# alibaba/animate-anything

Hardware: AMD Instinct MI355X
Metric: UNet3D denoising steps/sec @16fx512x512 bs=1 (higher is better)
Workload: dtype fp16; 1 GPU; animate_anything_512_v1.02 UNet3D (1413M params, seeded random init), 16 frames x 512x512, pipeline bs=1 per GPU (CFG batch 2, 17 frames inside), DPM-Solver++ step, hipGraph=on; clips_per_gpu=1, clips=1, parallelism=clip-sharded x1, collective=none

## Files before the change

### animate_anything_amd/_lib.py

```python
from __future__ import annotations

import ctypes as C
import os

import torch

AA_F16, AA_BF16, AA_F32 = 0, 1, 2
AA_ACT_NONE, AA_ACT_SILU, AA_ACT_GELU, AA_ACT_QUICK_GELU = 0, 1, 2, 3


class AaConvGemm(C.Structure):
    _fields_ = [
        ("a0", C.c_void_p), ("a1", C.c_void_p), ("w", C.c_void_p), ("bias", C.c_void_p),
        ("rowvec", C.c_void_p), ("residual", C.c_void_p), ("out", C.c_void_p),
        ("c0", C.c_int32), ("c1", C.c_int32),
        ("n_img", C.c_int32), ("h_in", C.c_int32), ("w_in", C.c_int32), ("h_virt", C.c_int32),
        ("w_virt", C.c_int32), ("h_out", C.c_int32), ("w_out", C.c_int32),
        ("kh", C.c_int32), ("kw", C.c_int32), ("stride", C.c_int32), ("pad_h", C.c_int32), ("pad_w", C.c_int32),
        ("n_out", C.c_int32), ("n_pad", C.c_int32), ("k_pad", C.c_int32),
        ("rowvec_div", C.c_int32), ("ldo", C.c_int32), ("ldr", C.c_int32),
        ("act", C.c_int32), ("geglu", C.c_int32), ("bias_per_row", C.c_int32),
        ("dtype", C.c_int32), ("out_dtype", C.c_int32), ("out_scale", C.c_float), ("workspace", C.c_void_p), ("workspace_bytes", C.c_int64), ("k_order", C.c_int32), ("debug", C.c_int32), ("tile", C.c_int32), ("k_splits", C.c_int32), ("rowvec_ld", C.c_int32), ("acc_scale", C.c_float),
        ("out_sy", C.c_int32), ("out_sx", C.c_int32), ("out_oy", C.c_int32), ("out_ox", C.c_int32),
        ("ln_stats", C.c_void_p), ("ln_cols", C.c_void_p), ("ln_parts", C.c_int32), ("ln_eps", C.c_float),
        ("row_stats", C.c_void_p), ("row_stats_parts", C.c_int32), ("tickets_len", C.c_int32), ("tickets", C.c_void_p),
        ("row_coef", C.c_void_p), ("row_coef_eps", C.c_float), ("_reserved107", C.c_int32),
    ]


class AaGroupNorm(C.Structure):
    _fields_ = [
        ("x0", C.c_void_p), ("x1", C.c_void_p), ("gamma", C.c_void_p), ("beta", C.c_void_p), ("y", C.c_void_p),
        ("c0", C.c_int32), ("c1", C.c_int32), ("n_groups_img", C.c_int32), ("tokens_per_group", C.c_int32),
        ("num_groups", C.c_int32), ("silu", C.c_int32), ("dtype", C.c_int32), ("eps", C.c_float),
    ]


class AaAttnOperand(C.Structure):
    _fields_ = [
        ("ptr", C.c_void_p), ("outer_stride", C.c_int64), ("inner_stride", C.c_int64), ("pos_stride", C.c_int64),
        ("ld", C.c_int32), ("col0", C.c_int32), ("outer_div", C.c_int32), ("seq_mod", C.c_int32),
    ]


class AaAttention(C.Structure):
    _fields_ = [
        ("q", AaAttnOperand), ("k", AaAttnOperand), ("v", AaAttnOperand), ("o", AaAttnOperand),
        ("n_outer", C.c_int32), ("n_inner", C.c_int32), ("heads", C.c_int32), ("head_dim", C.c_int32),
        ("q_len", C.c_int32), ("kv_len", C.c_int32), ("dtype", C.c_int32), ("scale", C.c_float), ("causal", C.c_int32), ("_pad", C.c_int32),
    ]


class AaSeqSelfAttn(C.Structure):
    _fields_ = [
        ("x", C.c_void_p), ("w", C.c_void_p), ("w_bias", C.c_void_p), ("pre_w", C.c_void_p), ("pre_bias", C.c_void_p), ("pre_residual", C.c_void_p), ("pre_out", C.c_void_p), ("o", C.c_void_p),
        ("outer_stride", C.c_int64), ("inner_stride", C.c_int64), ("pos_stride", C.c_int64), ("x_bytes", C.c_int64), ("o_bytes", C.c_int64),
        ("n_outer", C.c_int32), ("n_inner", C.c_int32), ("seq_len", C.c_int32), ("channels", C.c_int32), ("ldx", C.c_int32), ("ldo", C.c_int32), ("ld_res", C.c_int32), ("ld_pre", C.c_int32),
        ("normalize", C.c_int32), ("ln_eps", C.c_float), ("scale", C.c_float), ("dtype", C.c_int32), ("flags", C.c_int32),
    ]


class AaFFFused(C.Structure):
    _fields_ = [
        ("x", C.c_void_p), ("outer", C.c_void_p), ("out", C.c_void_p), ("w", C.c_void_p), ("rows", C.c_int64),
        ("channels", C.c_int32), ("ldx", C.c_int32), ("ld_outer", C.c_int32), ("ldo", C.c_int32),
        ("normalize", C.c_int32), ("ln_eps", C.c_float), ("dtype", C.c_int32), ("flags", C.c_int32),
    ]


class AaLinearRows(C.Structure):
    _fields_ = [
        ("x", C.c_void_p), ("residual", C.c_void_p), ("out", C.c_void_p), ("w", C.c_void_p), ("rows", C.c_int64),
        ("channels", C.c_int32), ("n_out", C.c_int32), ("ldx", C.c_int32), ("ld_res", C.c_int32), ("ldo", C.c_int32),
        ("normalize", C.c_int32), ("ln_eps", C.c_float), ("dtype", C.c_int32), ("flags", C.c_int32),
        ("row_affine", C.c_void_p), ("rows_per_group", C.c_int32), ("_pad", C.c_int32),
    ]


class AaQuantRowsFp8(C.Structure):
    _fields_ = [
        ("x", C.c_void_p), ("gamma", C.c_void_p), ("beta", C.c_void_p), ("q", C.c_void_p), ("scale", C.c_void_p), ("rows", C.c_int64),
        ("channels", C.c_int32), ("ldx", C.c_int32), ("ldq", C.c_int32), ("ln_eps", C.c_float), ("dtype", C.c_int32), ("_pad", C.c_int32),
    ]


class AaLinearFp8(C.Structure):
    _fields_ = [
        ("a", C.c_void_p), ("a_scale", C.c_void_p), ("w", C.c_void_p), ("w_scale", C.c_void_p), ("bias", C.c_void_p),
        ("residual", C.c_void_p), ("out", C.c_void_p), ("rows", C.c_int64),
        ("n", C.c_int32), ("k", C.c_int32), ("ld_res", C.c_int32), ("ldo", C.c_int32), ("geglu", C.c_int32), ("dtype", C.c_int32),
    ]


class AaDpmStep(C.Structure):
    _fields_ = [
        ("eps_uncond", C.c_void_p), ("eps_text", C.c_void_p), ("latents", C.c_void_p), ("x0_prev", C.c_void_p),
        ("latents_lp", C.c_void_p), ("n", C.c_int64),
        ("guidance", C.c_float), ("sigma_s", C.c_float), ("alpha_s", C.c_float),
        ("c_x", C.c_float), ("c_d0", C.c_float), ("c_d1", C.c_float), ("dtype", C.c_int32),
    ]


class AaPackLatents(C.Structure):
    _fields_ = [
        ("sample", C.c_void_p), ("cond", C.c_void_p), ("mask", C.c_void_p), ("out", C.c_void_p),
        ("batch", C.c_int32), ("sample_batch", C.c_int32), ("cond_batch", C.c_int32), ("mask_batch", C.c_int32),
        ("channels", C.c_int32), ("frames", C.c_int32), ("hw", C.c_int32), ("dtype", C.c_int32), ("sample_dtype", C.c_int32),
    ]


class AaDpmStepTok(C.Structure):
    _fields_ = [
        ("eps_tokens", C.c_void_p), ("latents", C.c_void_p), ("x0_prev", C.c_void_p), ("latents_lp", C.c_void_p),
        ("next_t", C.c_void_p), ("next_t_count", C.c_int32), ("next_t_value", C.c_float),
        ("clips", C.c_int32), ("channels", C.c_int32), ("frames", C.c_int32), ("hw", C.c_int32),
        ("eps_ld", C.c_int32), ("guidance_on", C.c_int32),
        ("guidance", C.c_float), ("sigma_s", C.c_float), ("alpha_s", C.c_float),
        ("c_x", C.c_float), ("c_d0", C.c_float), ("c_d1", C.c_float), ("dtype", C.c_int32),
    ]


class AaBlend(C.Structure):
    _fields_ = [
        ("x", C.c_void_p), ("y", C.c_void_p), ("rowvec", C.c_void_p), ("out", C.c_void_p), ("rows", C.c_int64),
        ("channels", C.c_int32), ("rowvec_div", C.c_int32), ("rowvec_mod", C.c_int32), ("rowvec_ld", C.c_int32),
        ("a", C.c_float), ("b", C.c_float), ("act", C.c_int32), ("dtype", C.c_int32),
    ]


class AaPackFrames(C.Structure):
    _fields_ = [
        ("src", C.c_void_p * 3), ("src_channels", C.c_int32 * 3), ("src_batch", C.c_int32 * 3), ("src_f32", C.c_int32 * 3),
        ("scale", C.c_void_p), ("scaled_src", C.c_int32), ("out", C.c_void_p),
        ("batch", C.c_int32), ("frames", C.c_int32), ("hw", C.c_int32), ("out_channels", C.c_int32), ("dtype", C.c_int32),
    ]


class AaEulerStepTok(C.Structure):
    _fields_ = [
        ("v_tokens", C.c_void_p), ("latents", C.c_void_p), ("guidance", C.c_void_p), ("next_t", C.c_void_p),
        ("next_t_count", C.c_int32), ("next_t_value", C.c_float), ("next_scale", C.c_void_p), ("next_scale_value", C.c_float),
        ("clips", C.c_int32), ("channels", C.c_int32), ("frames", C.c_int32), ("hw", C.c_int32), ("ld", C.c_int32),
        ("c_x", C.c_float), ("c_v", C.c_float), ("dtype", C.c_int32),
    ]


class AaDdimStepTok(C.Structure):
    _fields_ = [
        ("tokens", C.c_void_p), ("latents", C.c_void_p), ("latents_lp", C.c_void_p), ("noise", C.c_void_p), ("next_t", C.c_void_p),
        ("next_t_count", C.c_int32), ("next_t_value", C.c_float),
        ("clips", C.c_int32), ("channels", C.c_int32), ("frames", C.c_int32), ("hw", C.c_int32), ("ld", C.c_int32),
        ("guidance_on", C.c_int32), ("guidance", C.c_float), ("a_x", C.c_float), ("a_m", C.c_float),
        ("clip_on", C.c_int32), ("clip", C.c_float), ("eps_from_x0", C.c_int32),
        ("e_x", C.c_float), ("e_m", C.c_float), ("q_x", C.c_float), ("q_0", C.c_float),
        ("c_0", C.c_float), ("c_e", C.c_float), ("c_n", C.c_float), ("dtype", C.c_int32),
    ]


class AaUnipcStepTok(C.Structure):
    _fields_ = [
        ("tokens", C.c_void_p), ("latents", C.c_void_p), ("latents_lp", C.c_void_p), ("last_sample", C.c_void_p),
        ("hist1", C.c_void_p), ("hist2", C.c_void_p), ("hist3", C.c_void_p), ("next_t", C.c_void_p),
        ("next_t_count", C.c_int32), ("next_t_value", C.c_float),
        ("clips", C.c_int32), ("channels", C.c_int32), ("frames", C.c_int32), ("hw", C.c_int32), ("ld", C.c_int32),
        ("guidance_on", C.c_int32), ("guidance", C.c_float), ("a_x", C.c_float), ("a_m", C.c_float),
        ("corr_on", C.c_int32), ("q_l", C.c_float), ("q_1", C.c_float), ("q_2", C.c_float), ("q_3", C.c_float), ("q_n", C.c_float),
        ("p_x", C.c_float), ("p_0", C.c_float), ("p_1", C.c_float), ("p_2", C.c_float), ("dtype", C.c_int32),
    ]


class AaFreeU(C.Structure):
    _fields_ = [
        ("hidden", C.c_void_p), ("hidden_out", C.c_void_p), ("skip", C.c_void_p), ("skip_out", C.c_void_p), ("trig", C.c_void_p),
        ("images", C.c_int32), ("h", C.c_int32), ("w", C.c_int32), ("c_hidden", C.c_int32), ("c_skip", C.c_int32),
        ("hidden_ld", C.c_int32), ("hidden_out_ld", C.c_int32), ("skip_ld", C.c_int32), ("skip_out_ld", C.c_int32),
        ("b", C.c_float), ("s", C.c_float), ("dtype", C.c_int32),
    ]


# ... 115 lines not shown
```

### animate_anything_amd/csrc/aa_api_impl.h

```cpp
#pragma once
#include <stdarg.h>
#include <stdio.h>
#include <stdlib.h>
#include <string.h>
#include "aa_mi355.h"
#include "kernels/conv_gemm.h"
#include "kernels/conv_gemm_dma.h"
#include "kernels/conv_slab.h"
#include "kernels/conv_gemm_x.h"
#include "kernels/norm.h"
#include "kernels/attention.h"
#include "kernels/seq_attention.h"
#include "kernels/ff_fused.h"
#include "kernels/linear_rows.h"
#include "kernels/linear_fp8.h"
#include "kernels/glue.h"
#include "kernels/freeu.h"
#include "kernels/cfg_rescale.h"

namespace aa {

static thread_local char g_err[512] = "";

static int fail(int code, const char* fmt, ...) {
    va_list ap;
    va_start(ap, fmt);
    vsnprintf(g_err, sizeof(g_err), fmt, ap);
    va_end(ap);
    return code;
}

static int finish(const char* what) {
    const char* e = AA_POST_LAUNCH();
    if (e) return fail(AA_E_HIP, "%s: %s", what, e);
    return AA_OK;
}

static bool aligned16(const void* p) { return (reinterpret_cast<uintptr_t>(p) & 15) == 0; }

template <typename D>
static bool step_tok_geometry_ok(const D* d, int ld) {
    return d->clips > 0 && d->channels > 0 && d->frames > 0 && d->hw > 0 && ld >= d->channels && d->next_t_count >= 0 && d->next_t_count <= 256;
}

template <typename D>
static dim3 step_tok_grid(const D* d) {
    const int64_t blocks = ((int64_t)d->clips * d->channels * d->frames * d->hw + 255) / 256;
    return dim3((unsigned)(blocks > 2048 ? 2048 : blocks));
}

struct CgCfg { int bm, bn, wm, wn, bk, stages, per_cu; float rate; int slab = 0; int x = 0; int sched = 0; };
constexpr int cg_dp(int dp3, int dp0, int dp1) { return (dp3 | dp0 << 4 | dp1 << 8) << 6; }
static const CgCfg kCgCfgs[] = {
    {128, 64, 2, 2, 64, 2, 3, 0.78f},
    {128, 128, 2, 2, 64, 2, 2, 0.90f},
    {192, 256, 3, 2, 64, 2, 1, 1.05f},
    {256, 256, 4, 2, 64, 2, 1, 1.10f},
    {256, 320, 4, 2, 64, 2, 1, 1.10f},
    {192, 320, 3, 2, 64, 2, 1, 1.05f},
    {256, 320, 4, 2, 32, 4, 1, 1.15f},
    {256, 256, 4, 2, 32, 4, 1, 1.15f},
    {128, 128, 2, 2, 32, 4, 2, 0.95f},
    {128, 64, 2, 2, 32, 4, 3, 0.80f},
    {192, 320, 3, 2, 32, 4, 1, 1.10f},
    {128, 320, 2, 2, 32, 2, 2, 1.10f},
    {128, 256, 2, 2, 32, 2, 2, 1.05f},
    {128, 256, 2, 2, 64, 2, 1, 1.00f},
    {256, 320, 4, 2, 64, 2, 1, 1.30f, 0, 0, 1},
    {256, 256, 4, 2, 64, 2, 1, 1.25f, 0, 0, 1},
    {128, 128, 2, 2, 32, 2, 3, 0.90f},
    {128, 64, 2, 2, 32, 2, 4, 0.78f},
    {64, 128, 2, 2, 32, 2, 4, 0.70f},
    {64, 64, 2, 2, 32, 2, 6, 0.60f},
    {64, 256, 2, 2, 32, 2, 3, 0.80f},
    {256, 320, 4, 2, 32, 4, 1, 1.20f, 0, 0, 1},
    {256, 256, 4, 2, 32, 4, 1, 1.20f, 0, 0, 1},
    {192, 256, 2, 4, 64, 2, 1, 1.05f},
    {192, 256, 2, 4, 64, 2, 1, 1.05f, 0, 0, 1},
    {128, 256, 2, 4, 32, 2, 2, 1.00f},
    {256, 320, 4, 2, 64, 2, 1, 1.30f, 0, 0, 2},
    {256, 256, 4, 2, 64, 2, 1, 1.25f, 0, 0, 2},
    {192, 256, 2, 4, 64, 2, 1, 1.05f, 0, 0, 2},
    {256, 320, 4, 2, 32, 4, 1, 1.20f, 0, 0, 2},
    {128, 320, 2, 2, 32, 2, 2, 1.10f, 0, 0, 2},
    {128, 128, 2, 2, 64, 2, 2, 0.90f, 0, 0, 2},
    {192, 320, 3, 2, 64, 2, 1, 1.05f, 0, 0, 2},
    {128, 256, 2, 2, 32, 2, 2, 1.05f, 0, 0, 2},
    {256, 320, 4, 2, 32, 3, 1, 1.00f, 1},
    {256, 256, 4, 2, 32, 3, 1, 1.00f, 1},
    {256, 256, 2, 2, 64, 2, 1, 1.45f, 0, 1, cg_dp(8, 8, 0)},
    {256, 320, 2, 2, 64, 2, 1, 1.45f, 0, 1, cg_dp(11, 7, 0)},
    {256, 256, 2, 2, 64, 2, 1, 1.40f, 0, 1, cg_dp(6, 5, 5)},
    {256, 320, 2, 2, 64, 2, 1, 1.40f, 0, 1, cg_dp(7, 6, 5)},
    {256, 256, 4, 2, 64, 2, 1, 1.35f, 0, 1, cg_dp(2, 2, 2)},
    {256, 256, 2, 2, 32, 4, 1, 1.50f, 0, 1, cg_dp(4, 0, 0)},
    {256, 320, 2, 2, 32, 4, 1, 1.50f, 0, 1, cg_dp(5, 0, 0)},
    {256, 256, 4, 2, 32, 4, 1, 1.45f, 0, 1, cg_dp(2, 0, 0)},
    {128, 256, 2, 2, 32, 3, 2, 1.20f, 0, 1, cg_dp(3, 0, 0)},
    {256, 128, 4, 1, 32, 3, 2, 1.20f, 0, 1, cg_dp(3, 0, 0)},
    {192, 256, 2, 2, 64, 2, 1, 1.30f, 0, 1, cg_dp(5, 5, 4)},
    {128, 128, 2, 2, 64, 2, 2, 1.00f, 0, 1, cg_dp(2, 2, 2)},
    {128, 128, 2, 2, 32, 4, 2, 1.00f, 0, 1, cg_dp(2, 0, 0)},
    {192, 320, 2, 2, 64, 2, 1, 1.35f, 0, 1, cg_dp(6, 5, 5)},
};
constexpr int kNumCgCfgs = sizeof(kCgCfgs) / sizeof(kCgCfgs[0]);

static thread_local int g_tile_override = -2;
static int cg_force_cfg() {
    if (g_tile_override == -2) { const char* e = getenv("AA_FORCE_CFG"); g_tile_override = e ? atoi(e) : -1; }
    return g_tile_override;
}

static bool cg_slab_ok(const AaConvGemm& d, const CgCfg& c) {
    const int hw = d.h_in * d.w_in;
    return d.kh == 3 && d.kw == 3 && d.stride == 1 && d.pad_h == 1 && d.pad_w == 1 && d.h_virt == d.h_in && d.w_virt == d.w_in &&
           d.h_out == d.h_in && d.w_out == d.w_in && d.k_order == 1 && d.c0 % 64 == 0 && d.c1 % 64 == 0 && !d.geglu && !d.bias_per_row &&
           c.bm % d.w_in == 0 && hw % c.bm == 0 && (c.bm / d.w_in + 2) * (d.w_in + 2) <= CS_SLAB_ROWS && !(d.debug & 8);
}

static thread_local unsigned g_x_disabled = 0;
static bool cg_x_ok(const AaConvGemm& d) {
    if (!(d.h_virt == d.h_in && d.w_virt == d.w_in)) return false;
    {
        const int taps = d.kh * d.kw;
        if (taps > 1 && d.k_order != 1) return false;
        if (taps > 31) return false;
        const int64_t px = (int64_t)d.n_img * d.h_in * d.w_in + (int64_t)d.pad_h * d.w_in + d.pad_w + (int64_t)d.kh * d.w_in + d.kw;
        if (px >= ((int64_t)1 << 24) || px * (d.c0 > d.c1 ? d.c0 : d.c1) * 2 >= ((int64_t)1 << 31)) return false;
    }
    if (d.rowvec) {
        const int64_t M = (int64_t)d.n_img * d.h_out * d.w_out;
        const int64_t ld = d.rowvec_ld ? d.rowvec_ld : d.n_out;
        if (((M - 1) / (d.rowvec_div > 0 ? d.rowvec_div : 1) + 1) * ld * 2 >= ((int64_t)1 << 31)) return false;
    }
    return true;
}

static bool cg_tile_fits(const AaConvGemm& d, int i) {
    const CgCfg& c = kCgCfgs[i];
    if (d.n_pad % c.bn) return false;
    if (d.geglu && (c.bn / c.wn) % 64) return false;
    if (c.slab && !cg_slab_ok(d, c)) return false;
    if (c.x && (!cg_x_ok(d) || (i >= 36 && ((g_x_disabled >> (i - 36)) & 1u)))) return false;
    if (c.x && d.ln_stats && !cgx_ln_ok(c.bk, c.wm, c.wn, c.per_cu)) return false;
    return true;
}

static int cg_choose(const AaConvGemm& d, int M) {
    int best = -1;
    double best_cost = 0.0;
    const int forced = d.tile >= 0 ? d.tile : cg_force_cfg();
    for (int i = 0; i < kNumCgCfgs; ++i) {
        const CgCfg& c = kCgCfgs[i];
        if (!cg_tile_fits(d, i)) continue;
        if (forced == i) return i;
        const double tiles = (double)((M + c.bm - 1) / c.bm) * (d.n_pad / c.bn);
        const double slots = 256.0 * c.per_cu;
        const double rounds = (double)(long long)((tiles + slots - 1) / slots);
        const double cost = rounds * c.bm * c.bn * c.per_cu / c.rate;
        if (best < 0 || cost < best_cost) { best = i; best_cost = cost; }
    }
    return best;
}

static int cg_splits(const AaConvGemm& d, int M, const CgCfg& c) {
    if (d.geglu || c.slab) return 1;
    const int tiles = ((M + c.bm - 1) / c.bm) * (d.n_pad / c.bn);
    const int slots = 256 * c.per_cu;
    const int nk = d.k_pad / c.bk;
    if (d.k_splits >= 1) return d.k_splits <= nk ? d.k_splits : nk;
    if (tiles * 2 > slots || nk < 32) return 1;
    int s = slots / tiles;
    if (s > 8) s = 8;
    if (s > nk / 8) s = nk / 8;
    return s < 1 ? 1 : s;
}

static bool cg_dma_ok(const AaConvGemm& d) {
    const int n_cols = d.geglu ? d.n_out / 2 : d.n_out;
    return (d.c0 + d.c1) % 64 == 0 && d.c0 % 64 == 0 && d.kh <= 8 && d.kw <= 8 && d.out_dtype == d.dtype && n_cols % 8 == 0 &&
           d.ldo % 8 == 0 && aligned16(d.out) && (!d.residual || (d.ldr % 8 == 0 && aligned16(d.residual))) &&
           d.n_out % 8 == 0 && (!d.bias || d.bias_per_row || aligned16(d.bias)) && (!d.rowvec || aligned16(d.rowvec)) &&
           (int64_t)d.n_img * d.h_in * d.w_in * (d.c0 > d.c1 ? d.c0 : d.c1) * 2 < ((int64_t)1 << 31) &&
           (int64_t)d.n_pad * d.k_pad * 2 < ((int64_t)1 << 31) &&
           (!cgd_out_mapped(d) || (int64_t)d.n_img * d.h_out * d.w_out * (d.out_sy > 1 ? d.out_sy : 1) * (d.out_sx > 1 ? d.out_sx : 1) * d.ldo * 2 < ((int64_t)1 << 31) - 32);
}

struct CgPlan {
    int cfg;
    int splits;
    int m_main;
    int tail_cfg;
    int tail_splits;
    size_t workspace;
    int tickets;
};

static int cg_ticket_count(const AaConvGemm& d, int cfg, int m_begin, int M) {
    if (!d.tickets || cfg < 0 || !kCgCfgs[cfg].x || d.ln_stats || (d.debug & 8)) return 0;
    const CgCfg& c = kCgCfgs[cfg];
    if (!cgx_ticket_ok(c.bm, c.bn, c.wm, c.wn, c.per_cu)) return 0;
    const int wgs = ((M - m_begin + c.bm - 1) / c.bm) * (d.n_pad / c.bn);
    return wgs <= d.tickets_len ? wgs : 0;
}

static CgPlan cg_plan(const AaConvGemm& d, int M, bool have_workspace_or_query) {
    CgPlan p = {cg_choose(d, M), 1, M, -1, 1, 0, 0};
    if (p.cfg < 0) return p;
    const CgCfg& c = kCgCfgs[p.cfg];
    const bool probe = (d.debug & 8) != 0;
    if (probe) return p;
    p.splits = have_workspace_or_query ? cg_splits(d, M, c) : 1;
    if (p.splits > 1) { p.workspace = (size_t)p.splits * M * d.n_pad * 4; p.tickets = cg_ticket_count(d, p.cfg, 0, M); return p; }
    p.splits = 1;
    if (c.per_cu > 2) return p;
    const int tiles_n = d.n_pad / c.bn;
    const int tiles_m = (M + c.bm - 1) / c.bm;
    const int cus = ((d.debug & 4) ? 2 : 256) * c.per_cu;
    const int rounds = tiles_m * tiles_n / cus;
    const int rem = tiles_m * tiles_n - rounds * cus;
    if (!(rounds >= 1 && rem > 0 && rem * 8 < cus * 5)) return p;
    {
        const double t_round = (double)(d.k_pad / c.bk) * 1.3 * c.bm * c.bn / 65536.0 * (c.bk / 64.0) * c.per_cu + 8.0;
        if (!(d.debug & 4) && (1.0 - (double)rem / cus) * t_round < 25.0) return p;
    }
    p.m_main = (rounds * cus / tiles_n) * c.bm;
    if (p.m_main >= M) { p.m_main = M; return p; }
    const int nk = d.k_pad / c.bk;
    const int tail_tiles = ((M - p.m_main + c.bm - 1) / c.bm) * tiles_n;
    int ts = c.per_cu == 1 ? cus / tail_tiles : 1;
    if (ts > 8) ts = 8;
    if (ts > nk / 24) ts = nk / 24;
    if (have_workspace_or_query && ts >= 2 && !d.geglu) {
        p.tail_cfg = c.slab ? (c.bn == 320 ? 14 : 15) : p.cfg;
        p.tail_splits = ts;
        p.workspace = (size_t)ts * (M - p.m_main) * d.n_pad * 4;
        p.tickets = cg_ticket_count(d, p.tail_cfg, p.m_main, M);
        return p;
    }
    const int small[3] = {47, 1, 0};
    for (int k = 0; k < 3 && p.tail_cfg < 0; ++k)
        if (cg_tile_fits(d, small[k])) p.tail_cfg = small[k];
    if (p.tail_cfg < 0) p.tail_cfg = p.cfg;
    return p;
}

template <typename T, int BM, int BN, int WM, int WN, int BK, int STAGES, int PER_CU, bool STAGGER = false, bool SPREAD = false>
static void cg_launch_dma(const AaConvGemm& d, int m_begin, int m_end, int splits, void* stream) {
    const int tiles_n = d.n_pad / BN;
    const dim3 grid(((m_end - m_begin + BM - 1) / BM) * tiles_n, splits), block(64 * WM * WN);
    AA_LAUNCH((conv_gemm_dma_kernel<T, BM, BN, WM, WN, BK, STAGES, PER_CU, STAGGER, SPREAD>), grid, block, cgd_lds_bytes(BM, BN, BK, STAGES), stream, d, m_end, tiles_n, m_begin, splits);
}

template <typename T, int BM, int BN, int WM, int WN>
static void cg_launch_slab(const AaConvGemm& d, int m_begin, int m_end, void* stream) {
    const int tiles_n = d.n_pad / BN;
    const dim3 grid(((m_end - m_begin) / BM) * tiles_n), block(64 * WM * WN);
    AA_LAUNCH((conv3x3_slab_kernel<T, BM, BN, WM, WN>), grid, block, cs_lds_bytes(BN), stream, d, m_end, tiles_n, m_begin);
}

template <typename T, int BM, int BN, int WM, int WN, int BK, int DP3, int DP0, int DP1, int RING = (BK == 64 ? 2 : 4), int PER_CU = 1>
static void cg_launch_x(const AaConvGemm& d, int m_begin, int m_end, int splits, void* stream) {
    const int tiles_n = d.n_pad / BN;
    const dim3 grid(((m_end - m_begin + BM - 1) / BM) * tiles_n, splits), block(64 * WM * WN);
    if (d.kh * d.kw == 1 && d.stride == 1 && d.pad_h == 0 && d.pad_w == 0)
        AA_LAUNCH((conv_gemm_x_kernel<T, BM, BN, WM, WN, BK, DP3, DP0, DP1, RING, PER_CU, true>), grid, block, cgx_lds_bytes(BM, BN, BK, RING, WM, WN, PER_CU), stream, d, m_end, tiles_n, m_begin, splits);
    else
        AA_LAUNCH((conv_gemm_x_kernel<T, BM, BN, WM, WN, BK, DP3, DP0, DP1, RING, PER_CU, false>), grid, block, cgx_lds_bytes(BM, BN, BK, RING, WM, WN, PER_CU), stream, d, m_end, tiles_n, m_begin, splits);
}

#ifndef AA_TU_GROUPS
#define AA_TU_GROUPS 1
#endif
template <typename T, int G>
bool cg_launch_cfg_group(int cfg, const AaConvGemm& d, int m_begin, int m_end, void* stream, int splits) {
#define AA_TILE(i, ...) case i: if constexpr (i % AA_TU_GROUPS == G) { __VA_ARGS__; return true; } else return false;
    switch (cfg) {
        AA_TILE(0, cg_launch_dma<T, 128, 64, 2, 2, 64, 2, 3>(d, m_begin, m_end, splits, stream))
        AA_TILE(1, cg_launch_dma<T, 128, 128, 2, 2, 64, 2, 2>(d, m_begin, m_end, splits, stream))
        AA_TILE(2, cg_launch_dma<T, 192, 256, 3, 2, 64, 2, 1>(d, m_begin, m_end, splits, stream))
        AA_TILE(3, cg_launch_dma<T, 256, 256, 4, 2, 64, 2, 1>(d, m_begin, m_end, splits, stream))
        AA_TILE(4, cg_launch_dma<T, 256, 320, 4, 2, 64, 2, 1>(d, m_begin, m_end, splits, stream))
        AA_TILE(5, cg_launch_dma<T, 192, 320, 3, 2, 64, 2, 1>(d, m_begin, m_end, splits, stream))
        AA_TILE(6, cg_launch_dma<T, 256, 320, 4, 2, 32, 4, 1>(d, m_begin, m_end, splits, stream))
        AA_TILE(7, cg_launch_dma<T, 256, 256, 4, 2, 32, 4, 1>(d, m_begin, m_end, splits, stream))
        AA_TILE(8, cg_launch_dma<T, 128, 128, 2, 2, 32, 4, 2>(d, m_begin, m_end, splits, stream))
        AA_TILE(9, cg_launch_dma<T, 128, 64, 2, 2, 32, 4, 3>(d, m_begin, m_end, splits, stream))
        AA_TILE(10, cg_launch_dma<T, 192, 320, 3, 2, 32, 4, 1>(d, m_begin, m_end, splits, stream))
        AA_TILE(11, cg_launch_dma<T, 128, 320, 2, 2, 32, 2, 2>(d, m_begin, m_end, splits, stream))
        AA_TILE(12, cg_launch_dma<T, 128, 256, 2, 2, 32, 2, 2>(d, m_begin, m_end, splits, stream))
        AA_TILE(13, cg_launch_dma<T, 128, 256, 2, 2, 64, 2, 1>(d, m_begin, m_end, splits, stream))
        AA_TILE(14, cg_launch_dma<T, 256, 320, 4, 2, 64, 2, 1, true>(d, m_begin, m_end, splits, stream))
        AA_TILE(15, cg_launch_dma<T, 256, 256, 4, 2, 64, 2, 1, true>(d, m_begin, m_end, splits, stream))
        AA_TILE(16, cg_launch_dma<T, 128, 128, 2, 2, 32, 2, 3>(d, m_begin, m_end, splits, stream))
        AA_TILE(17, cg_launch_dma<T, 128, 64, 2, 2, 32, 2, 4>(d, m_begin, m_end, splits, stream))
        AA_TILE(18, cg_launch_dma<T, 64, 128, 2, 2, 32, 2, 4>(d, m_begin, m_end, splits, stream))
        AA_TILE(19, cg_launch_dma<T, 64, 64, 2, 2, 32, 2, 6>(d, m_begin, m_end, splits, stream))
        AA_TILE(20, cg_launch_dma<T, 64, 256, 2, 2, 32, 2, 3>(d, m_begin, m_end, splits, stream))
        AA_TILE(21, cg_launch_dma<T, 256, 320, 4, 2, 32, 4, 1, true>(d, m_begin, m_end, splits, stream))
        AA_TILE(22, cg_launch_dma<T, 256, 256, 4, 2, 32, 4, 1, true>(d, m_begin, m_end, splits, stream))
        AA_TILE(23, cg_launch_dma<T, 192, 256, 2, 4, 64, 2, 1>(d, m_begin, m_end, splits, stream))
        AA_TILE(24, cg_launch_dma<T, 192, 256, 2, 4, 64, 2, 1, true>(d, m_begin, m_end, splits, stream))
        AA_TILE(25, cg_launch_dma<T, 128, 256, 2, 4, 32, 2, 2>(d, m_begin, m_end, splits, stream))
        AA_TILE(26, cg_launch_dma<T, 256, 320, 4, 2, 64, 2, 1, false, true>(d, m_begin, m_end, splits, stream))
        AA_TILE(27, cg_launch_dma<T, 256, 256, 4, 2, 64, 2, 1, false, true>(d, m_begin, m_end, splits, stream))
        AA_TILE(28, cg_launch_dma<T, 192, 256, 2, 4, 64, 2, 1, false, true>(d, m_begin, m_end, splits, stream))
        AA_TILE(29, cg_launch_dma<T, 256, 320, 4, 2, 32, 4, 1, false, true>(d, m_begin, m_end, splits, stream))
        AA_TILE(30, cg_launch_dma<T, 128, 320, 2, 2, 32, 2, 2, false, true>(d, m_begin, m_end, splits, stream))
        AA_TILE(31, cg_launch_dma<T, 128, 128, 2, 2, 64, 2, 2, false, true>(d, m_begin, m_end, splits, stream))
        AA_TILE(32, cg_launch_dma<T, 192, 320, 3, 2, 64, 2, 1, false, true>(d, m_begin, m_end, splits, stream))
        AA_TILE(33, cg_launch_dma<T, 128, 256, 2, 2, 32, 2, 2, false, true>(d, m_begin, m_end, splits, stream))
        AA_TILE(34, cg_launch_slab<T, 256, 320, 4, 2>(d, m_begin, m_end, stream))
        AA_TILE(35, cg_launch_slab<T, 256, 256, 4, 2>(d, m_begin, m_end, stream))
        AA_TILE(36, cg_launch_x<T, 256, 256, 2, 2, 64, 8, 8, 0>(d, m_begin, m_end, splits, stream))
        AA_TILE(37, cg_launch_x<T, 256, 320, 2, 2, 64, 11, 7, 0>(d, m_begin, m_end, splits, stream))
        AA_TILE(38, cg_launch_x<T, 256, 256, 2, 2, 64, 6, 5, 5>(d, m_begin, m_end, splits, stream))
        AA_TILE(39, cg_launch_x<T, 256, 320, 2, 2, 64, 7, 6, 5>(d, m_begin, m_end, splits, stream))
        AA_TILE(40, cg_launch_x<T, 256, 256, 4, 2, 64, 2, 2, 2>(d, m_begin, m_end, splits, stream))
        AA_TILE(41, cg_launch_x<T, 256, 256, 2, 2, 32, 4, 0, 0>(d, m_begin, m_end, splits, stream))
        AA_TILE(42, cg_launch_x<T, 256, 320, 2, 2, 32, 5, 0, 0>(d, m_begin, m_end, splits, stream))
        AA_TILE(43, cg_launch_x<T, 256, 256, 4, 2, 32, 2, 0, 0>(d, m_begin, m_end, splits, stream))
        AA_TILE(44, cg_launch_x<T, 128, 256, 2, 2, 32, 3, 0, 0, 3, 2>(d, m_begin, m_end, splits, stream))
        AA_TILE(45, cg_launch_x<T, 256, 128, 4, 1, 32, 3, 0, 0, 3, 2>(d, m_begin, m_end, splits, stream))
        AA_TILE(46, cg_launch_x<T, 192, 256, 2, 2, 64, 5, 5, 4>(d, m_begin, m_end, splits, stream))
        AA_TILE(47, cg_launch_x<T, 128, 128, 2, 2, 64, 2, 2, 2, 2, 2>(d, m_begin, m_end, splits, stream))
        AA_TILE(48, cg_launch_x<T, 128, 128, 2, 2, 32, 2, 0, 0, 4, 2>(d, m_begin, m_end, splits, stream))
        AA_TILE(49, cg_launch_x<T, 192, 320, 2, 2, 64, 6, 5, 5>(d, m_begin, m_end, splits, stream))
        default: return false;
    }
#undef AA_TILE
}
#if AA_TU_GROUPS > 1
#define AA_X(g) extern template bool cg_launch_cfg_group<f16_t, g>(int, const AaConvGemm&, int, int, void*, int); \
                extern template bool cg_launch_cfg_group<bf16_t, g>(int, const AaConvGemm&, int, int, void*, int);
AA_X(0) AA_X(1) AA_X(2) AA_X(3) AA_X(4) AA_X(5) AA_X(6) AA_X(7)
#undef AA_X
static_assert(AA_TU_GROUPS == 8, "aa_tiles.hip is compiled once per group: keep build.py and this list in step");
#endif

template <typename T>
static bool cg_launch_cfg(int cfg, const AaConvGemm& d, int m_begin, int m_end, void* stream, int splits = 1) {
    if (cfg < 0) return false;
#if AA_TU_GROUPS > 1
    switch (cfg % AA_TU_GROUPS) {
        case 0: return cg_launch_cfg_group<T, 0>(cfg, d, m_begin, m_end, stream, splits);
        case 1: return cg_launch_cfg_group<T, 1>(cfg, d, m_begin, m_end, stream, splits);
        case 2: return cg_launch_cfg_group<T, 2>(cfg, d, m_begin, m_end, stream, splits);
        case 3: return cg_launch_cfg_group<T, 3>(cfg, d, m_begin, m_end, stream, splits);
        case 4: return cg_launch_cfg_group<T, 4>(cfg, d, m_begin, m_end, stream, splits);
        case 5: return cg_launch_cfg_group<T, 5>(cfg, d, m_begin, m_end, stream, splits);
        case 6: return cg_launch_cfg_group<T, 6>(cfg, d, m_begin, m_end, stream, splits);
        default: return cg_launch_cfg_group<T, 7>(cfg, d, m_begin, m_end, stream, splits);
    }
#else
    return cg_launch_cfg_group<T, 0>(cfg, d, m_begin, m_end, stream, splits);
#endif
}

#ifdef AA_TU_TILES_ONLY
}
#else
template <typename T>
static int conv_gemm_t(const AaConvGemm& d, void* stream) {
    const int M = (int)((int64_t)d.n_img * d.h_out * d.w_out);
    if (cg_dma_ok(d)) {
        CgPlan pl = cg_plan(d, M, d.workspace != nullptr);
        if (pl.cfg < 0) return fail(AA_E_SHAPE, "conv_gemm: no tile shape divides n_pad=%d (geglu=%d)", d.n_pad, d.geglu);
        if (pl.workspace > (size_t)d.workspace_bytes) pl = cg_plan(d, M, false);
        auto reduce = [&](int m_begin, int splits) {
            int64_t blocks = ((int64_t)(M - m_begin) * (d.n_out / 8) + 255) / 256;
            if (blocks > 4096) blocks = 4096;
            AA_LAUNCH((splitk_reduce_kernel<T>), dim3((unsigned)blocks), dim3(256), 0, stream, d, M, m_begin, splits);
        };
        AaConvGemm dk = d;
        if (!pl.tickets) dk.tickets = nullptr;
        if (pl.splits > 1) {
            cg_launch_cfg<T>(pl.cfg, dk, 0, M, stream, pl.splits);
            if (!pl.tickets) reduce(0, pl.splits);
            return finish("conv_gemm");
        }
        cg_launch_cfg<T>(pl.cfg, dk, 0, pl.m_main, stream);
        if (pl.m_main < M) {
            AaConvGemm tail = dk;
            tail.tile = -1;
            cg_launch_cfg<T>(pl.tail_cfg, tail, pl.m_main, M, stream, pl.tail_splits);
            if (pl.tail_splits > 1 && !pl.tickets) reduce(pl.m_main, pl.tail_splits);
        }
        return finish("conv_gemm");
    }
    if (d.geglu) return fail(AA_E_SHAPE, "conv_gemm: GEGLU needs the LDS-DMA path (channels %% 64 == 0, 16-byte rows)");
    if (d.k_order) return fail(AA_E_SHAPE, "conv_gemm: chunk-major weights need the LDS-DMA path (channels %% 64 == 0, 16-byte rows)");
    const bool bn128 = (d.n_pad % 128 == 0);
    const int bn = bn128 ? 128 : 64;
    const int tiles_n = d.n_pad / bn;
    const dim3 grid(((M + CG_BM - 1) / CG_BM) * tiles_n), block(CG_THREADS);
    if (bn128) AA_LAUNCH((conv_gemm_kernel<T, 128>), grid, block, cg_lds_bytes(128), stream, d, M, tiles_n);
    else       AA_LAUNCH((conv_gemm_kernel<T, 64>), grid, block, cg_lds_bytes(64), stream, d, M, tiles_n);
    return finish("conv_gemm");
}

template <typename T>
static int groupnorm_t(const AaGroupNorm& d, float* ws, int chunks, int apply_chunks, void* stream) {
    const int C = d.c0 + d.c1;
    const int S = C / 8;
    const int rpp = S <= GN_THREADS ? GN_THREADS / S : 1;
    AA_LAUNCH((groupnorm_stats_kernel<T>), dim3(chunks, d.n_groups_img), dim3(GN_THREADS), (size_t)C * 8 * (1 + rpp), stream, d, ws, chunks);
    const size_t lds = ((size_t)2 * C + 2 * (GN_THREADS + d.num_groups)) * 4;
    AA_LAUNCH((groupnorm_apply_kernel<T>), dim3(apply_chunks, d.n_groups_img), dim3(GN_THREADS), lds, stream, d, (const float*)ws, chunks, apply_chunks);
    return finish("groupnorm");
}

struct GnfPlan { int gb, nr, parts, grid; };
static bool gnf_plan(const AaGroupNorm& d, GnfPlan& best) {
    const int C = d.c0 + d.c1, G = d.num_groups, cg = C / G;
    static const int kNR[] = {8, 16, 24, 32, 48};
    bool found = false;
    long best_est = 0;
    for (int gb = 1; gb <= G; gb *= 2) {
// ... 33 lines not shown
}

static thread_local bool g_gn_two_pass = false;
static int gn_chunks(const AaGroupNorm& d) {
    int want = 1024 / d.n_groups_img;
    if (want < 1) want = 1;
    int cap = (d.tokens_per_group + 15) / 16;
    if (cap > 256) cap = 256;
    int c = want < cap ? want : cap;
    return c < 1 ? 1 : c;
}

template <typename T>
static int attention_t(const AaAttention& d, void* stream) {
    const int nseq = d.n_outer * d.n_inner;
    if (d.head_dim == 8 || d.head_dim == 80) {
        const dim3 grid((d.q_len + 255) / 256, d.heads, nseq);
        const size_t lds = (size_t)2 * 256 * d.head_dim * sizeof(T);
        if (d.head_dim == 8) AA_LAUNCH((attention_small_kernel<T, 8>), grid, dim3(256), lds, stream, d);
        else                 AA_LAUNCH((attention_small_kernel<T, 80>), grid, dim3(256), lds, stream, d);
        return finish("attention");
    }
    if (d.q_len >= 128 && d.kv_len > AT_KT && d.kv_len <= ATS_KEYS && !d.causal && !(d._pad & 4)) {
        const int n_qb = (d.q_len + 31) / 32;
        int qb = 8;
        while (qb > 1 && (int64_t)((n_qb + 4 * qb - 1) / (4 * qb)) * d.heads * nseq < 1024) qb >>= 1;
        const dim3 grid((n_qb + 4 * qb - 1) / (4 * qb), d.heads, nseq);
        AA_LAUNCH((attention_shortkv_kernel<T>), grid, dim3(256), 2 * AT_TILE_BYTES, stream, d, qb);
    } else if (d.q_len >= 512 && d.kv_len >= 512 && (d._pad & 8)) {
        const dim3 grid((d.q_len + 255) / 256, d.heads, nseq);
        AA_LAUNCH((attention_kernel<T, 4, 64, 1, 2>), grid, dim3(256), attn_lds_bytes(d.kv_len), stream, d);
    } else if (d.q_len > 64) {
        const dim3 grid((d.q_len + 127) / 128, d.heads, nseq);
        AA_LAUNCH((attention_kernel<T, 4>), grid, dim3(256), attn_lds_bytes(d.kv_len), stream, d);
    } else {
        const dim3 grid((d.q_len + 31) / 32, d.heads, nseq);
        if (d.kv_len <= 32 && d.q_len <= 32 && nseq >= 4096) {
            const dim3 grid8(1, d.heads, (nseq + 7) / 8);
            AA_LAUNCH((attention_kernel<T, 1, 32, 8>), grid8, dim3(512), 8 * (AT_TILE_BYTES / 2), stream, d);
        } else if (d.kv_len <= 32 && d.q_len <= 32 && nseq >= 256) {
            const dim3 grid4(1, d.heads, (nseq + 3) / 4);
            AA_LAUNCH((attention_kernel<T, 1, 32, 4>), grid4, dim3(256), 4 * (AT_TILE_BYTES / 2), stream, d);
        } else if (d.kv_len <= 32) AA_LAUNCH((attention_kernel<T, 1, 32>), grid, dim3(64), AT_TILE_BYTES / 2, stream, d);
        else                AA_LAUNCH((attention_kernel<T, 1>), grid, dim3(64), attn_lds_bytes(d.kv_len), stream, d);
    }
    return finish("attention");
}

}

extern "C" {

int aa_version(void) { return AA_VERSION; }
int aa_conv_gemm_tile_info(int idx, int32_t info[7]) {
    if (idx < 0 || idx >= aa::kNumCgCfgs || !info) return -1;
    const aa::CgCfg& c = aa::kCgCfgs[idx];
    info[0] = c.bm; info[1] = c.bn; info[2] = c.wm; info[3] = c.wn; info[4] = c.bk; info[5] = c.stages; info[6] = c.per_cu;
    return 0;
}
int aa_conv_gemm_tile_ok(const AaConvGemm* d, int idx) {
    using namespace aa;
    if (!d || idx < 0 || idx >= kNumCgCfgs || !cg_dma_ok(*d)) return 0;
    return cg_tile_fits(*d, idx) ? 1 : 0;
}
void aa_set_tile_override(int cfg) {
    if (cfg <= -100) { aa::g_x_disabled = (unsigned)(-100 - cfg); return; }
    aa::g_tile_override = cfg < 0 ? -1 : cfg;
}
const char* aa_last_error(void) { return aa::g_err; }

size_t aa_conv_gemm_workspace(const AaConvGemm* d) {
    using namespace aa;
    if (!d || !cg_dma_ok(*d)) return 0;
    const int M = (int)((int64_t)d->n_img * d->h_out * d->w_out);
    return cg_plan(*d, M, true).workspace;
}

int aa_conv_gemm_row_stats_parts(const AaConvGemm* d) {
    using namespace aa;
    if (!d || !cg_dma_ok(*d) || d->geglu || d->rowvec || d->act != AA_ACT_NONE || d->bias_per_row || d->ln_stats || cgd_out_mapped(*d)) return 0;
    const int M = (int)((int64_t)d->n_img * d->h_out * d->w_out);
    CgPlan pl = cg_plan(*d, M, d->workspace != nullptr);
    if (pl.cfg < 0) return 0;
    if (pl.workspace > (size_t)d->workspace_bytes) pl = cg_plan(*d, M, false);
    const CgCfg& c = kCgCfgs[pl.cfg];
    if (!c.x || (pl.splits > 1 && !pl.tickets) || pl.m_main < M || (d->debug & 8)) return 0;
    return (d->n_pad / c.bn) * c.wn;
}

int aa_conv_gemm_row_coef_ok(const AaConvGemm* d) {
    using namespace aa;
    if (!d || !cg_dma_ok(*d)) return 0;
    AaConvGemm q = *d;
    q.row_coef = nullptr;
    const int parts = aa_conv_gemm_row_stats_parts(&q);
    if (parts <= 0) return 0;
    const int M = (int)((int64_t)d->n_img * d->h_out * d->w_out);
    CgPlan pl = cg_plan(q, M, q.workspace != nullptr);
    if (pl.workspace > (size_t)q.workspace_bytes) pl = cg_plan(q, M, false);
    const CgCfg& c = kCgCfgs[pl.cfg];
    return (d->n_pad == c.bn && parts == c.wn && pl.splits == 1 && pl.m_main >= M && c.wm * c.wn * (c.bm / c.wm) * 8 <= CGX_COEF_BYTES) ? 1 : 0;
}

static bool cg_plan_of(const AaConvGemm* d, aa::CgPlan& pl, int& M) {
    using namespace aa;
    if (!d || !cg_dma_ok(*d)) return false;
    M = (int)((int64_t)d->n_img * d->h_out * d->w_out);
    pl = cg_plan(*d, M, d->workspace != nullptr);
    if (pl.cfg < 0) return false;
    if (pl.workspace > (size_t)d->workspace_bytes) pl = cg_plan(*d, M, false);
    return true;
}

int aa_conv_gemm_reduce_launches(const AaConvGemm* d) {
    aa::CgPlan pl; int M;
    if (!cg_plan_of(d, pl, M) || pl.tickets) return 0;
    if (pl.splits > 1) return 1;
    return (pl.m_main < M && pl.tail_splits > 1) ? 1 : 0;
}

int aa_conv_gemm_tickets(const AaConvGemm* d) {
    aa::CgPlan pl; int M;
    if (!d) return 0;
    AaConvGemm q = *d;
    static int32_t probe_array;
    if (!q.tickets) { q.tickets = &probe_array; q.tickets_len = 0x7fffffff; }
    if (!cg_plan_of(&q, pl, M)) return 0;
    return pl.tickets;
}

int aa_conv_gemm_launch_count(const AaConvGemm* d) {
    using namespace aa;
    if (!d) return 0;
    if (!cg_dma_ok(*d)) return 1;
    CgPlan pl; int M;
    if (!cg_plan_of(d, pl, M)) return 0;
    int n = 1;
    if (pl.splits == 1 && pl.m_main < M) n += 1;
    return n + aa_conv_gemm_reduce_launches(d);
}

int aa_conv_gemm_tile_flags(int idx) {
    if (idx < 0 || idx >= aa::kNumCgCfgs) return -1;
    const aa::CgCfg& c = aa::kCgCfgs[idx];
    return (c.slab ? 1 : 0) | (c.x ? 2 : 0) | (c.sched << 2);
}

int aa_conv_gemm(const AaConvGemm* d, void* stream) {
    using namespace aa;
    if (!d) return fail(AA_E_SHAPE, "conv_gemm: null descriptor");
    const int ctot = d->c0 + d->c1;
    if (d->c0 <= 0 || d->c0 % 8 || d->c1 % 8 || (d->c1 > 0 && !d->a1))
        return fail(AA_E_SHAPE, "conv_gemm: channels must be multiples of 8 (c0=%d c1=%d)", d->c0, d->c1);
    if (d->n_pad % 64 || d->k_pad % CG_BK || d->k_pad < d->kh * d->kw * ctot || d->n_out > d->n_pad)
        return fail(AA_E_SHAPE, "conv_gemm: bad packed extents n_pad=%d k_pad=%d (K=%d, n_out=%d)", d->n_pad, d->k_pad, d->kh * d->kw * ctot, d->n_out);
    if (d->n_img <= 0 || d->h_out <= 0 || d->w_out <= 0 || d->kh <= 0 || d->kw <= 0 || d->stride <= 0 || d->rowvec_div <= 0)
        return fail(AA_E_SHAPE, "conv_gemm: bad geometry");
    if (d->rowvec_ld < 0 || d->rowvec_ld % 8 || (d->rowvec_ld && d->rowvec_ld < d->n_out)) return fail(AA_E_SHAPE, "conv_gemm: rowvec_ld=%d must be 0 or a multiple of 8 >= n_out", d->rowvec_ld);
    if (d->geglu && (d->geglu != 32 || d->n_out != d->n_pad || d->bias_per_row))
        return fail(AA_E_SHAPE, "conv_gemm: GEGLU packs (32 value | 32 gate) column blocks, n_out == n_pad (geglu=%d n_out=%d)", d->geglu, d->n_out);
    if ((int64_t)d->n_img * d->h_out * d->w_out >= (int64_t)1 << 31) return fail(AA_E_SHAPE, "conv_gemm: M overflows int32");
    if (!aligned16(d->a0) || !aligned16(d->a1) || !aligned16(d->w)) return fail(AA_E_ALIGN, "conv_gemm: operands must be 16-byte aligned");
    if (d->out_dtype != AA_F32 && d->out_dtype != d->dtype) return fail(AA_E_DTYPE, "conv_gemm: out_dtype must be dtype or f32");
    if (d->act != AA_ACT_NONE && d->act != AA_ACT_SILU) return fail(AA_E_SHAPE, "conv_gemm: activation %d is not fused here (AA_ACT_NONE / AA_ACT_SILU)", d->act);
    if (d->out_sy < 0 || d->out_sx < 0 || d->out_oy < 0 || d->out_ox < 0 || d->out_oy >= (d->out_sy > 1 ? d->out_sy : 1) || d->out_ox >= (d->out_sx > 1 ? d->out_sx : 1))
        return fail(AA_E_SHAPE, "conv_gemm: bad output grid mapping (out_sy=%d out_sx=%d out_oy=%d out_ox=%d)", d->out_sy, d->out_sx, d->out_oy, d->out_ox);
    if (d->ln_stats) {
        if (!d->ln_cols || d->bias || d->rowvec || d->residual || d->act != AA_ACT_NONE || d->bias_per_row || d->c1 ||
            d->kh * d->kw != 1 || d->out_scale != 1.0f || (d->acc_scale != 0.0f && d->acc_scale != 1.0f) || !cg_dma_ok(*d) || cgd_out_mapped(*d))
            return fail(AA_E_SHAPE, "conv_gemm: the LayerNorm fold (ln_stats) is a plain or GEGLU linear call: ln_cols, no bias / row vector / residual / activation / scales");
        if (d->ln_parts < 0 || d->ln_parts > 64 || (d->ln_parts > 0 && !(d->ln_eps > 0.0f)))
            return fail(AA_E_SHAPE, "conv_gemm: ln_parts=%d (0: finalised coefficients, 1..64: raw partial sums + ln_eps > 0)", d->ln_parts);
    }
    if (d->row_coef) {
        if (d->row_stats || d->row_stats_parts || !(d->row_coef_eps > 0.0f) || !aligned16(d->row_coef) || !aa_conv_gemm_row_coef_ok(d))
            return fail(AA_E_SHAPE, "conv_gemm: row_coef needs a statistics-emitting call whose tile spans the output row (aa_conv_gemm_row_coef_ok), "
                                    "row_stats NULL, row_coef_eps > 0, 16-byte aligned coefficients");
    }
    if (d->row_stats && d->row_stats_parts != aa_conv_gemm_row_stats_parts(d))
        return fail(AA_E_SHAPE, "conv_gemm: row_stats_parts=%d, this call emits %d partial statistics per row (aa_conv_gemm_row_stats_parts)", d->row_stats_parts, aa_conv_gemm_row_stats_parts(d));
    if (cgd_out_mapped(*d) && !cg_dma_ok(*d)) return fail(AA_E_SHAPE, "conv_gemm: a scattered output grid needs the LDS-DMA path (channels %% 64, 16-byte rows, < 2 GiB)");
    if (d->tile >= 0 && !aa_conv_gemm_tile_ok(d, d->tile))
        return fail(AA_E_SHAPE, "conv_gemm: tile %d (AaConvGemm.tile) cannot carry out this call (aa_conv_gemm_tile_ok == 0)", d->tile);
    if (d->dtype == AA_F16) return conv_gemm_t<f16_t>(*d, stream);
    if (d->dtype == AA_BF16) return conv_gemm_t<bf16_t>(*d, stream);
    return fail(AA_E_DTYPE, "conv_gemm: unsupported dtype %d", d->dtype);
}

size_t aa_groupnorm_workspace(const AaGroupNorm* d) {
    return (size_t)d->n_groups_img * aa::gn_chunks(*d) * d->num_groups * 2 * sizeof(float);
}

void aa_set_groupnorm_two_pass(int on) { aa::g_gn_two_pass = on != 0; }
int aa_groupnorm_plan(const AaGroupNorm* d, int32_t info[4]) {
    aa::GnfPlan pl;
    if (!d || !info || aa::g_gn_two_pass || !aa::gnf_plan(*d, pl)) return 0;
    info[0] = pl.gb; info[1] = pl.nr; info[2] = pl.parts; info[3] = pl.grid;
    return 1;
}

int aa_groupnorm(const AaGroupNorm* d, void* workspace, size_t workspace_bytes, void* stream) {
    using namespace aa;
    if (!d) return fail(AA_E_SHAPE, "groupnorm: null descriptor");
    const int C = d->c0 + d->c1;
    if (d->c0 <= 0 || d->c0 % 8 || d->c1 % 8 || d->num_groups <= 0 || C % d->num_groups || d->num_groups > GN_THREADS)
        return fail(AA_E_SHAPE, "groupnorm: bad channels c0=%d c1=%d groups=%d", d->c0, d->c1, d->num_groups);
    if (d->n_groups_img <= 0 || d->tokens_per_group <= 0) return fail(AA_E_SHAPE, "groupnorm: bad token geometry");
    if (!aligned16(d->x0) || !aligned16(d->x1) || !aligned16(d->y)) return fail(AA_E_ALIGN, "groupnorm: operands must be 16-byte aligned");
    const size_t need = aa_groupnorm_workspace(d);
    if (!workspace || workspace_bytes < need) return fail(AA_E_WORKSPACE, "groupnorm: workspace %zu < %zu bytes", workspace_bytes, need);
    if (d->dtype != AA_F16 && d->dtype != AA_BF16) return fail(AA_E_DTYPE, "groupnorm: unsupported dtype %d", d->dtype);
    GnfPlan pl;
    if (!g_gn_two_pass && gnf_plan(*d, pl)) {
        if (d->dtype == AA_F16) gnf_launch<f16_t>(*d, pl, stream);
        else gnf_launch<bf16_t>(*d, pl, stream);
        return finish("groupnorm");
    }
    const int chunks = gn_chunks(*d);
    if (d->dtype == AA_F16) return groupnorm_t<f16_t>(*d, (float*)workspace, chunks, chunks, stream);
    return groupnorm_t<bf16_t>(*d, (float*)workspace, chunks, chunks, stream);
}

int aa_groupnorm_coef(const AaGroupNorm* d, void* workspace, size_t workspace_bytes, float* coef, void* stream) {
    using namespace aa;
    if (!d || !coef) return fail(AA_E_SHAPE, "groupnorm_coef: null descriptor / coef");
    const int C = d->c0 + d->c1;
    if (d->c0 <= 0 || d->c0 % 8 || d->c1 % 8 || d->num_groups <= 0 || C % d->num_groups || d->num_groups > GN_THREADS)
        return fail(AA_E_SHAPE, "groupnorm_coef: bad channels c0=%d c1=%d groups=%d", d->c0, d->c1, d->num_groups);
    if (d->n_groups_img <= 0 || d->tokens_per_group <= 0) return fail(AA_E_SHAPE, "groupnorm_coef: bad token geometry");
    if (d->silu) return fail(AA_E_SHAPE, "groupnorm_coef: a norm with SiLU behind it is not affine");
    if (!aligned16(d->x0) || !aligned16(d->x1) || !aligned16(coef)) return fail(AA_E_ALIGN, "groupnorm_coef: operands must be 16-byte aligned");
    const size_t need = aa_groupnorm_workspace(d);
    if (!workspace || workspace_bytes < need) return fail(AA_E_WORKSPACE, "groupnorm_coef: workspace %zu < %zu bytes", workspace_bytes, need);
    if (d->dtype != AA_F16 && d->dtype != AA_BF16) return fail(AA_E_DTYPE, "groupnorm_coef: unsupported dtype %d", d->dtype);
    const int chunks = gn_chunks(*d), S = C / 8, rpp = S <= GN_THREADS ? GN_THREADS / S : 1;
    const size_t lds = (size_t)2 * (GN_THREADS + d->num_groups) * 4;
    float* ws = (float*)workspace;
    if (d->dtype == AA_F16) {
        AA_LAUNCH((groupnorm_stats_kernel<f16_t>), dim3(chunks, d->n_groups_img), dim3(GN_THREADS), (size_t)C * 8 * (1 + rpp), stream, *d, ws, chunks);
        AA_LAUNCH((groupnorm_coef_kernel<f16_t>), dim3(d->n_groups_img), dim3(GN_THREADS), lds, stream, *d, (const float*)ws, chunks, coef);
    } else {
        AA_LAUNCH((groupnorm_stats_kernel<bf16_t>), dim3(chunks, d->n_groups_img), dim3(GN_THREADS), (size_t)C * 8 * (1 + rpp), stream, *d, ws, chunks);
        AA_LAUNCH((groupnorm_coef_kernel<bf16_t>), dim3(d->n_groups_img), dim3(GN_THREADS), lds, stream, *d, (const float*)ws, chunks, coef);
    }
    return finish("groupnorm_coef");
}

int aa_layernorm(const void* x, const void* gamma, const void* beta, void* y, int64_t rows, int32_t channels,
                 float eps, int32_t dtype, void* stream) {
    using namespace aa;
    if (rows <= 0 || channels <= 0 || channels % 8 || channels > 2048) return fail(AA_E_SHAPE, "layernorm: rows=%lld channels=%d", (long long)rows, channels);
    if (!aligned16(x) || !aligned16(y) || !aligned16(gamma) || !aligned16(beta)) return fail(AA_E_ALIGN, "layernorm: operands must be 16-byte aligned");
    const int sj = channels <= 512 ? 1 : (channels <= 1024 ? 2 : 4);
    const int per_wg = 4 * (4 / sj);
    const dim3 grid((unsigned)((rows + per_wg - 1) / per_wg)), block(256);
    if (dtype != AA_F16 && dtype != AA_BF16) return fail(AA_E_DTYPE, "layernorm: unsupported dtype %d", dtype);
#define AA_LN(T, SJ) AA_LAUNCH((layernorm_kernel<T, SJ>), grid, block, 0, stream, (const T*)x, (const T*)gamma, (const T*)beta, (T*)y, rows, channels, eps)
    if (dtype == AA_F16) { if (sj == 1) AA_LN(f16_t, 1); else if (sj == 2) AA_LN(f16_t, 2); else AA_LN(f16_t, 4); }
    else                 { if (sj == 1) AA_LN(bf16_t, 1); else if (sj == 2) AA_LN(bf16_t, 2); else AA_LN(bf16_t, 4); }
#undef AA_LN
    return finish("layernorm");
}

int aa_ln_finalize(const float* stats, int32_t parts, float* coef, int64_t rows, int32_t channels, float eps, void* stream) {
    using namespace aa;
    if (!stats || !coef || parts <= 0 || rows <= 0 || channels <= 0) return fail(AA_E_SHAPE, "ln_finalize: rows=%lld parts=%d channels=%d", (long long)rows, parts, channels);
    if (!aligned16(coef)) return fail(AA_E_ALIGN, "ln_finalize: coef must be 16-byte aligned");
    const dim3 grid((unsigned)((rows + 255) / 256)), block(256);
    AA_LAUNCH(ln_finalize_kernel<0>, grid, block, 0, stream, stats, coef, rows, (int)parts, 1.0f / (float)channels, eps);
    return finish("ln_finalize");
}

int aa_attention(const AaAttention* d, void* stream) {
    using namespace aa;
    if (!d) return fail(AA_E_SHAPE, "attention: null descriptor");
    if (d->head_dim != 64 && d->head_dim != 8 && d->head_dim != 80) return fail(AA_E_SHAPE, "attention: head_dim must be 64, 8 or 80 (got %d)", d->head_dim);
    if (d->q_len <= 0 || d->kv_len <= 0 || d->heads <= 0 || d->n_outer <= 0 || d->n_inner <= 0) return fail(AA_E_SHAPE, "attention: bad lengths");
    const AaAttnOperand* ops[4] = {&d->q, &d->k, &d->v, &d->o};
    for (const AaAttnOperand* x : ops) {
        if (!aligned16(x->ptr) || x->ld % 8 || x->col0 % 8) return fail(AA_E_ALIGN, "attention: operand rows must be 16-byte aligned");
        if (x->outer_div <= 0) return fail(AA_E_SHAPE, "attention: outer_div must be >= 1");
        if (x->seq_mod < 0) return fail(AA_E_SHAPE, "attention: seq_mod must be >= 0");
    }
    if (d->q.seq_mod || d->o.seq_mod) return fail(AA_E_SHAPE, "attention: seq_mod addressing is for K / V only");
    if (d->causal && d->head_dim != 64) return fail(AA_E_SHAPE, "attention: causal masking is implemented for head_dim 64");
    if (d->head_dim == 64 && (attn_extent_bytes(d->k, d->n_outer, d->n_inner, d->kv_len) >= ((int64_t)1 << 31) ||
        attn_extent_bytes(d->v, d->n_outer, d->n_inner, d->kv_len) >= ((int64_t)1 << 31)))
        return fail(AA_E_SHAPE, "attention: K / V operand must stay below 2 GiB");
    if (d->dtype == AA_F16) return attention_t<f16_t>(*d, stream);
    if (d->dtype == AA_BF16) return attention_t<bf16_t>(*d, stream);
    return fail(AA_E_DTYPE, "attention: unsupported dtype %d", d->dtype);
}

int aa_seq_self_attention_ok(const AaSeqSelfAttn* d) {
    using namespace aa;
    if (!d) return 0;
    if (d->channels != 320 && d->channels != 512 && d->channels != 640) return 0;
    if (d->seq_len < 1 || d->seq_len > 32 || d->n_outer <= 0 || d->n_inner <= 0) return 0;
    if (d->ldx % 8 || d->ldo % 8 || d->ldx < d->channels || d->ldo < d->channels) return 0;
    if (d->x_bytes <= 0 || d->o_bytes <= 0 || d->x_bytes >= ((int64_t)1 << 31) || d->o_bytes >= ((int64_t)1 << 31)) return 0;
    if (d->dtype != AA_F16 && d->dtype != AA_BF16) return 0;
    return 1;
}

int aa_seq_self_attention(const AaSeqSelfAttn* d, void* stream) {
    using namespace aa;
// ... 370 lines not shown
```

### animate_anything_amd/csrc/kernels/conv_gemm_dma.h

```cpp
#pragma once
#include "dev.h"
#include "aa_mi355.h"
#include "conv_gemm.h"

namespace aa {

__host__ __device__ inline int cgd_lds_bytes(int bm, int bn, int bk, int stages) {
    return stages * (bm + bn) * bk * 2 + 1024 + 1024;
}

__host__ __device__ __forceinline__ bool cgd_out_mapped(const AaConvGemm& p) { return p.out_sy > 1 || p.out_sx > 1; }
__host__ __device__ __forceinline__ int64_t cgd_out_row(const AaConvGemm& p, const int m) {
    if (!cgd_out_mapped(p)) return m;
    const int sy = p.out_sy > 1 ? p.out_sy : 1, sx = p.out_sx > 1 ? p.out_sx : 1;
    const int x = m % p.w_out, t = m / p.w_out, y = t % p.h_out, img = t / p.h_out;
    return ((int64_t)img * (p.h_out * sy) + (y * sy + p.out_oy)) * (p.w_out * sx) + (x * sx + p.out_ox);
}

struct LnRow { float a, nm, nmean, sd; };
template <int MI> struct LnRstd { float v[MI]; bool on; };
__device__ __forceinline__ LnRow cgd_ln_row(const AaConvGemm& p, const int m) {
    if (p.ln_parts > 0) {
        const float* st = p.ln_stats + (int64_t)m * (p.ln_parts * 2);
        float s = 0.0f, q = 0.0f;
// ... 238 lines not shown
        } else {
            if (post) cgd_epilogue_fast<T, MI, NI, false, false, true, !BIAS_FOLDED, false, false>(p, M, get, m_wave, n_wave, sBiasW, part, ln_rstd);
            else cgd_epilogue_fast<T, MI, NI, false, false, false, !BIAS_FOLDED, false, false>(p, M, get, m_wave, n_wave, sBiasW, part, ln_rstd);
            return;
        }
    }
#define AA_ZERO4 (u32x4{0u, 0u, 0u, 0u})
    auto col_of = [&](int j) __attribute__((always_inline)) { return p.geglu ? (n_wave >> 1) + (j >> 1) * 32 + 16 * eh : n_wave + j * 32 + 16 * eh; };
    static_for<MI>([&](auto i_) __attribute__((always_inline)) {
        constexpr int i = decltype(i_)::value;
        const int m = m_wave + i * 32 + ec;
        const bool m_ok = m < M;
        const int mc = m_ok ? m : M - 1;
        const float brow = (p.bias_per_row && bias) ? (float)bias[mc] : 0.0f;
        const T* rv = rowvec ? rowvec + (int64_t)(mc / p.rowvec_div) * (p.rowvec_ld ? p.rowvec_ld : p.n_out) : nullptr;
        const T* rs = resid ? resid + (int64_t)mc * p.ldr : nullptr;
        const int64_t o_row_g = cgd_out_row(p, mc) * p.ldo;
        const LnRow lr = lnf ? cgd_ln_row(p, mc) : LnRow{1.0f, 0.0f, 0.0f, 1.0f};
        u32x4 pre[NI][2];
#pragma unroll
        for (int j = 0; j < NI; ++j)
#pragma unroll
            for (int q = 0; q < 2; ++q) {
                const int n_rv = n_wave + j * 32 + 16 * eh + 8 * q, n_rs = col_of(j) + 8 * q;
                const bool ok = pre_is_rv ? (n_rv + 8 <= p.n_out) : (rs != nullptr && !(p.geglu && (j & 1)) && n_rs + 8 <= n_cols);
                const T* src = pre_is_rv ? rv + n_rv : rs + n_rs;
                pre[j][q] = ok ? *reinterpret_cast<const u32x4*>(src) : AA_ZERO4;
            }
        auto finish_block = [&](int j, float (&v)[2][8]) __attribute__((always_inline)) {
            const int nc = col_of(j);
#pragma unroll
            for (int q = 0; q < 2; ++q) {
                const u32x4 pv = pre[j][q];
                if (post) {
                    Pack8<T> r; r.raw = AA_ZERO4;
                    if (rs) { if (pre_is_rv) { if (nc + 8 * q + 8 <= n_cols) r.raw = *reinterpret_cast<const u32x4*>(rs + nc + 8 * q); } else r.raw = pv; }
#pragma unroll
                    for (int e = 0; e < 8; ++e) v[q][e] = (v[q][e] * acc_scale + (float)r.e[e]) * p.out_scale;
                }
                Pack8<T> o;
#pragma unroll
                for (int e = 0; e < 8; ++e) o.e[e] = (T)v[q][e];
                if ((AA_X_ABLATE & 16) ? (o.raw[0] == 0x12345678u && m_ok) : (m_ok && nc + 8 * q + 8 <= n_cols)) *reinterpret_cast<u32x4*>(out + o_row_g + nc + 8 * q) = o.raw;
            }
        };
        auto block_f32 = [&](auto j_, float (&v)[2][8]) __attribute__((always_inline)) {
            constexpr int j = decltype(j_)::value;
            const f32x16 a = get(IntTag<i>(), IntTag<j>());
#pragma unroll
            for (int q = 0; q < 2; ++q) {
                Pack8<T> b; b.raw = *reinterpret_cast<const u32x4*>(sBiasW + (j * 32 + 16 * eh + 8 * q));
                const u32x4 pv = pre[j][q];
                Pack8<T> r; r.raw = AA_ZERO4;
                if (pre_is_rv) r.raw = pv;
#pragma unroll
                for (int e = 0; e < 8; ++e) v[q][e] = a[8 * q + e] + (float)b.e[e] + brow;
                if (lnf && !ln_rstd.on) {
                    const float* cs = p.ln_cols + n_wave + j * 32 + 16 * eh + 8 * q;
#pragma unroll
                    for (int e = 0; e < 8; ++e) v[q][e] = fmaf(v[q][e], lr.a, fmaf(lr.nm, cs[e], cs[p.n_pad + e]));
                }
                if (pre_is_rv) {
#pragma unroll
                    for (int e = 0; e < 8; ++e) v[q][e] += (float)r.e[e];
                }
                if (silu) {
#pragma unroll
                    for (int e = 0; e < 8; ++e) v[q][e] = silu_f(v[q][e]);
                }
            }
        };
        if (p.geglu) {
            if constexpr (NI % 2 == 0) {
                static_for<NI / 2>([&](auto h_) __attribute__((always_inline)) {
                    constexpr int j = 2 * decltype(h_)::value;
                    float val[2][8], gate[2][8];
                    block_f32(IntTag<j>(), val);
                    block_f32(IntTag<j + 1>(), gate);
#pragma unroll
                    for (int q = 0; q < 2; ++q)
#pragma unroll
                        for (int e = 0; e < 8; ++e) val[q][e] *= (AA_X_ABLATE & 8) ? gate[q][e] : gelu_erf_f(gate[q][e]);
                    finish_block(j, val);
                });
            }
        } else {
            static_for<NI>([&](auto j_) __attribute__((always_inline)) {
                float v[2][8];
                block_f32(j_, v);
                finish_block(decltype(j_)::value, v);
            });
        }
    });
#undef AA_ZERO4
}

template <typename T, int MI, int NI>
__device__ __forceinline__ void cgd_epilogue(const AaConvGemm& p, const int M, f32x16 (&acc)[MI][NI], const int m_wave, const int n_wave,
                                             const T* sBiasW) {
    cgd_epilogue_g<T, MI, NI, false>(p, M, [&](auto i_, auto j_) __attribute__((always_inline)) -> const f32x16& { return acc[decltype(i_)::value][decltype(j_)::value]; },
                              m_wave, n_wave, sBiasW);
}

template <typename T, int BM, int BN, int WM, int WN, int BK, int STAGES, int PER_CU, bool STAGGER, bool SPREAD = false>
__global__ void __launch_bounds__(64 * WM * WN, (PER_CU * WM * WN + 3) / 4) conv_gemm_dma_kernel(const AaConvGemm p, const int M, const int tiles_n, const int m_begin, const int k_splits) {
    constexpr int NW = WM * WN;
    constexpr int THREADS = 64 * NW;
    constexpr int MI = BM / WM / 32;
    constexpr int NI = BN / WN / 32;
    constexpr int ROWB = BK * 2;
    constexpr int SPR = BK / 8;
    constexpr int RPI = 64 / SPR;
    constexpr int RPB = 256 / ROWB;
    constexpr int GA = BM / RPI, GB = BN / RPI;
    constexpr int AJ = (GA + NW - 1) / NW;
    constexpr int BJ = (GB + NW - 1) / NW;
    constexpr int PER_TILE = AJ + BJ;
    constexpr int DIST = STAGES - 1;
    constexpr int STAGE_BYTES = (BM + BN) * ROWB;
    constexpr bool FRAG_ASM = (MI * NI * 16 + 2 * (MI + NI) * 4) <= 184;
    static_assert(BM % (32 * WM) == 0 && BN % (32 * WN) == 0 && BM % RPI == 0 && BN % RPI == 0, "tile shape");
    static_assert(BK == 64 || BK == 32, "K step");
    static_assert(STAGES >= 2 && STAGES <= 4 && (STAGES - 2) * PER_TILE <= 63, "pipeline depth");
    char* smem = dyn_smem();
    char* dummy = smem + STAGES * STAGE_BYTES;
    T* sBias = reinterpret_cast<T*>(dummy + 1024);
    static_assert(BN * 2 <= 1024, "bias slice");

    const int tid = threadIdx.x;
    const int lane = tid & 63;
    const int wave = wave_id();
    const int wm = wave / WN, wn = wave % WN;

    const int nwg = gridDim.x, bid = blockIdx.x;
    const int q = nwg >> 3, r = nwg & 7;
    const int xcd = bid & 7, idx = bid >> 3;
    const int logical = (xcd < r ? xcd * (q + 1) : r * (q + 1) + (xcd - r) * q) + idx;
    const int tile_m = logical / tiles_n;
    const int tile_n = logical - tile_m * tiles_n;

    auto stamp = [&](int slot) {
        if ((p.debug & 8) && tid == 0) reinterpret_cast<long long*>(p.workspace)[(int64_t)blockIdx.x * 8 + slot] = clock_now();
    };
    stamp(0);
    const int ctot = p.c0 + p.c1;
    const int nk_all = p.k_pad / BK;
    const int k_per = (nk_all + k_splits - 1) / k_splits;
    const int kbase = blockIdx.y * k_per;
    const int nk = max(0, min(k_per, nk_all - kbase));
    const bool resize = (p.h_virt != p.h_in) || (p.w_virt != p.w_in);
    const bool linear = p.kh * p.kw == 1 && p.stride == 1 && p.pad_h == 0 && p.pad_w == 0 && !resize;

    constexpr unsigned OOB = 0x80000000u;
    const BufRsrc r_a0 = make_rsrc(p.a0, (unsigned)((int64_t)p.n_img * p.h_in * p.w_in * p.c0 * 2));
    const BufRsrc r_a1 = make_rsrc(p.a1, p.c1 ? (unsigned)((int64_t)p.n_img * p.h_in * p.w_in * p.c1 * 2) : 0u);
    const BufRsrc r_w = make_rsrc(p.w, (unsigned)((int64_t)p.n_pad * p.k_pad * 2));
#ifdef AA_PHASE_PROBE
    const int swm = (p.debug & 16) ? 0 : SPR - 1;
    const bool dry = p.debug & 32;
#else
    constexpr int swm = SPR - 1;
    constexpr bool dry = false;
#endif
    const bool two_src = p.c1 != 0;
    const int lrow = lane / SPR, lpos = lane % SPR;
    unsigned ctr0[AJ], ctr1[AJ], vmask[AJ];
    struct RowCoords { int img, iy, ix; bool ok; };
    auto row_coords = [&](int j) __attribute__((always_inline)) {
        const int rr = (wave + NW * j) * RPI + lrow;
        const int m = m_begin + tile_m * BM + rr;
        const bool ok = m < M && rr < BM;
        const int mm = ok ? m : 0;
        if (linear) return RowCoords{0, 0, mm, ok};
        const int x = mm % p.w_out;
        const int t = mm / p.w_out;
        const int y = t % p.h_out;
        return RowCoords{t / p.h_out, y * p.stride - p.pad_h, x * p.stride - p.pad_w, ok};
    };
#pragma unroll
    for (int j = 0; j < AJ; ++j) {
        const RowCoords rc = row_coords(j);
        const int img = rc.img, iy = rc.iy, ix = rc.ix;
        const bool ok = rc.ok;
        const int rr = (wave + NW * j) * RPI + lrow;
        const int slot8 = (lpos ^ ((rr / RPB) & swm)) * 8;
        const int pix = (img * p.h_in + iy) * p.w_in + ix;
        ctr0[j] = (unsigned)(pix * p.c0 + slot8) * 2u;
        ctr1[j] = (unsigned)(pix * p.c1 + slot8) * 2u;
        const int ylo = max(0, -iy), yhi = max(ylo, min(p.kh, p.h_virt - iy));
        const int xlo = max(0, -ix), xhi = max(xlo, min(p.kw, p.w_virt - ix));
        const unsigned my = ((1u << yhi) - 1u) ^ ((1u << ylo) - 1u), mx = ((1u << xhi) - 1u) ^ ((1u << xlo) - 1u);
        vmask[j] = ok ? (my | (mx << 8)) : 0u;
    }
    unsigned wb[BJ];
#pragma unroll
    for (int j = 0; j < BJ; ++j) {
        const int rr = (wave + NW * j) * RPI + lrow;
        wb[j] = (unsigned)((tile_n * BN + rr) * p.k_pad + (lpos ^ ((rr / RPB) & swm)) * 8) * 2u;
    }

    const int taps = p.kh * p.kw;

    int n_tap, n_dy, n_dx, n_cb;
    {
        const int k0 = kbase * BK;
        if (p.k_order) { const int unit = k0 >> 6; const int chunk = unit / taps; n_tap = unit - chunk * taps; n_cb = chunk * 64 + (k0 & 63); }
        else           { n_tap = k0 / ctot; n_cb = k0 - n_tap * ctot; }
        n_dy = n_tap / p.kw; n_dx = n_tap - n_dy * p.kw;
    }
    int cur_tap = -1;
    unsigned pb0[AJ], pb1[AJ];
    bool is_src1 = false;
    unsigned is_ccb = 0u, is_kb = 0u;
    int is_buf = 0;
    auto issue_prepare = [&](int kt, int buf) {
        const int tap = n_tap, cb = n_cb, dy = n_dy, dx = n_dx;
        {
            const bool wrap_x = n_dx + 1 == p.kw;
            if (p.k_order) {
                const bool half = BK == 32 && !(n_cb & 32);
                const bool last_tap = n_tap + 1 == taps;
                const int cb_unit = (n_cb & ~63) + (last_tap ? 64 : 0);
                const int t1 = last_tap ? 0 : n_tap + 1;
                const int y1 = last_tap ? 0 : (wrap_x ? n_dy + 1 : n_dy);
                const int x1 = (last_tap || wrap_x) ? 0 : n_dx + 1;
                n_cb = half ? n_cb + 32 : cb_unit;
                n_tap = half ? n_tap : t1; n_dy = half ? n_dy : y1; n_dx = half ? n_dx : x1;
            } else {
                const bool last_c = n_cb + BK >= ctot;
                n_cb = last_c ? 0 : n_cb + BK;
                n_tap = last_c ? n_tap + 1 : n_tap;
                n_dy = (last_c && wrap_x) ? n_dy + 1 : n_dy;
                n_dx = last_c ? (wrap_x ? 0 : n_dx + 1) : n_dx;
            }
        }
        if (tap != cur_tap) {
            cur_tap = tap;
            const bool tap_ok = tap < taps;
            if (!resize) {
                const int d = dy * p.w_in + dx;
                const unsigned d0 = (unsigned)(d * p.c0) * 2u;
#pragma unroll
                for (int j = 0; j < AJ; ++j) {
                    const bool ok = tap_ok && (((vmask[j] >> dy) & (vmask[j] >> (8 + dx))) & 1u);
                    pb0[j] = ok ? ctr0[j] + d0 : OOB;
                }
                if (two_src) {
                    const unsigned d1 = (unsigned)(d * p.c1) * 2u;
#pragma unroll
                    for (int j = 0; j < AJ; ++j) {
                        const bool ok = tap_ok && (((vmask[j] >> dy) & (vmask[j] >> (8 + dx))) & 1u);
                        pb1[j] = ok ? ctr1[j] + d1 : OOB;
                    }
                }
            } else {
#pragma unroll
                for (int j = 0; j < AJ; ++j) {
                    const bool ok = tap_ok && (((vmask[j] >> dy) & (vmask[j] >> (8 + dx))) & 1u);
                    const RowCoords rc = row_coords(j);
                    const int sy = ((rc.iy + dy) * p.h_in) / p.h_virt, sx = ((rc.ix + dx) * p.w_in) / p.w_virt;
                    const int pix = (rc.img * p.h_in + sy) * p.w_in + sx;
                    const int rr = (wave + NW * j) * RPI + lrow;
                    const int slot8 = (lpos ^ ((rr / RPB) & swm)) * 8;
                    pb0[j] = ok ? (unsigned)(pix * p.c0 + slot8) * 2u : OOB;
                    pb1[j] = ok ? (unsigned)(pix * p.c1 + slot8) * 2u : OOB;
                }
            }
        }
        is_src1 = cb >= p.c0;
        is_ccb = (unsigned)(is_src1 ? cb - p.c0 : cb) * 2u;
        is_kb = (unsigned)((kbase + kt) * BK) * 2u;
        is_buf = buf;
    };
    auto issue_dma = [&](auto j0_, auto j1_) {
        constexpr int J0 = decltype(j0_)::value, J1 = decltype(j1_)::value;
        const BufRsrc ra = is_src1 ? r_a1 : r_a0;
        char* a = smem + is_buf * STAGE_BYTES + wave * RPI * ROWB;
        char* b = smem + is_buf * STAGE_BYTES + BM * ROWB + wave * RPI * ROWB;
#pragma unroll
        for (int jj = J0; jj < J1; ++jj) {
            if (jj < AJ) {
                const int j = jj;
                const bool real = (GA % NW == 0) || (wave + NW * j < GA);
                async_copy16_buf(ra, (real && !dry) ? (is_src1 ? pb1[j] : pb0[j]) + is_ccb : OOB, real ? a + j * NW * RPI * ROWB : dummy);
            } else {
                const int j = jj - AJ;
                const bool real = (GB % NW == 0) || (wave + NW * j < GB);
                async_copy16_buf(r_w, (real && !dry) ? wb[j] + is_kb : OOB, real ? b + j * NW * RPI * ROWB : dummy);
            }
        }
    };
    auto issue = [&](int kt, int buf) {
        issue_prepare(kt, buf);
        issue_dma(IntTag<0>(), IntTag<PER_TILE>());
    };

    f32x16 acc[MI][NI];
#pragma unroll
    for (int i = 0; i < MI; ++i)
#pragma unroll
        for (int j = 0; j < NI; ++j)
#pragma unroll
            for (int e = 0; e < 16; ++e) acc[i][j][e] = 0.0f;

    const int frow = lane & 31, fh = lane >> 5;
    int a_off[MI], b_off[NI], a_swz[MI], b_swz[NI];
#pragma unroll
    for (int i = 0; i < MI; ++i) { const int rr = wm * (BM / WM) + i * 32 + frow; a_off[i] = rr * ROWB; a_swz[i] = (rr / RPB) & swm; }
    const int prow = (frow & 3) + 4 * (frow >> 3) + 16 * ((frow >> 2) & 1);
#pragma unroll
    for (int j = 0; j < NI; ++j) { const int rr = wn * (BN / WN) + j * 32 + prow; b_off[j] = BM * ROWB + rr * ROWB; b_swz[j] = (rr / RPB) & swm; }

    auto frag_ptr_a = [&](const char* st, int ks, int i) { return st + a_off[i] + (((ks * 2 + fh) ^ a_swz[i]) << 4); };
    auto frag_ptr_b = [&](const char* st, int ks, int j) { return st + b_off[j] + (((ks * 2 + fh) ^ b_swz[j]) << 4); };
    constexpr int KS = BK / 16;
    constexpr int SP = (KS >= 4 && STAGES == 2) ? KS - 1 : KS;
    auto issue_piece = [&](auto ks_, int kt_next) {
        constexpr int ks = decltype(ks_)::value;
        if constexpr (ks < SP) {
            constexpr int J0 = PER_TILE * ks / SP, J1 = PER_TILE * (ks + 1) / SP;
            issue_dma(IntTag<J0>(), IntTag<J1>());
        }
    };
    auto compute = [&](int buf, int issue_at, int kt_next, bool more) {
        const char* st = smem + buf * STAGE_BYTES;
        if constexpr (FRAG_ASM) {
            u32x4 fa[2][MI], fb[2][NI];
            auto issue_frags = [&](int ks, int set) {
#pragma unroll
                for (int i = 0; i < MI; ++i) lds_read16_async(fa[set][i], frag_ptr_a(st, ks, i));
#pragma unroll
                for (int j = 0; j < NI; ++j) lds_read16_async(fb[set][j], frag_ptr_b(st, ks, j));
            };
            issue_frags(0, 0);
            auto substep = [&](auto ks_) __attribute__((always_inline)) {
                constexpr int ks = decltype(ks_)::value;
                constexpr int set = ks & 1;
                if constexpr (SPREAD) { if (more) issue_piece(ks_, kt_next); }
                else if (more && ks == issue_at) issue(kt_next, kt_next % STAGES);
                if constexpr (ks + 1 < KS) { issue_frags(ks + 1, set ^ 1); lds_wait<MI + NI>(fa[set][0]); }
                else lds_wait<0>(fa[set][0]);
#pragma unroll
                for (int i = 1; i < MI; ++i) lds_pin(fa[set][i]);
#pragma unroll
                for (int j = 0; j < NI; ++j) lds_pin(fb[set][j]);
#pragma unroll
                for (int i = 0; i < MI; ++i)
#pragma unroll
                    for (int j = 0; j < NI; ++j) acc[i][j] = mfma_32x32x16(T(), fb[set][j], fa[set][i], acc[i][j]);
            };
            substep(IntTag<0>());
            substep(IntTag<1>());
            if constexpr (KS == 4) { substep(IntTag<2>()); substep(IntTag<3>()); }
        } else {
            auto piece = [&](auto ks_) __attribute__((always_inline)) { if constexpr (SPREAD) { if (more) issue_piece(ks_, kt_next); } };
#pragma unroll
            for (int ks = 0; ks < KS; ++ks) {
                if constexpr (SPREAD) {
                    if (ks == 0) piece(IntTag<0>());
                    if (ks == 1) piece(IntTag<1>());
                    if (KS == 4 && ks == 2) piece(IntTag<2>());
                    if (KS == 4 && ks == 3) piece(IntTag<3>());
                } else if (more && ks == issue_at) issue(kt_next, kt_next % STAGES);
                u32x4 fa[MI], fb[NI];
#pragma unroll
                for (int i = 0; i < MI; ++i) fa[i] = *reinterpret_cast<const u32x4*>(frag_ptr_a(st, ks, i));
#pragma unroll
                for (int j = 0; j < NI; ++j) fb[j] = *reinterpret_cast<const u32x4*>(frag_ptr_b(st, ks, j));
#pragma unroll
                for (int i = 0; i < MI; ++i)
#pragma unroll
                    for (int j = 0; j < NI; ++j) acc[i][j] = mfma_32x32x16(T(), fb[j], fa[i], acc[i][j]);
            }
        }
    };

#ifdef AA_PHASE_PROBE
    long long pt[4] = {0, 0, 0, 0};
    long long plast = clock_now();
#define AA_TICK(k) { const long long now_ = clock_now(); pt[k] += now_ - plast; plast = now_; }
#else
#define AA_TICK(k)
#endif
    stamp(1);
    {
#pragma unroll
        for (int t = 0; t < DIST; ++t)
            if (t < nk) issue(t, t);
        if constexpr (SPREAD) { if (DIST < nk) issue_prepare(DIST, DIST % STAGES); }
        if (tid < BN / 8) {
            const int n = tile_n * BN + tid * 8;
            u32x4 b = u32x4{0u, 0u, 0u, 0u};
            if (p.bias && !p.bias_per_row && n + 8 <= p.n_out) b = *reinterpret_cast<const u32x4*>(reinterpret_cast<const T*>(p.bias) + n);
            *reinterpret_cast<u32x4*>(sBias + tid * 8) = b;
        }
        for (int kt = 0; kt < nk; ++kt) {
            const int younger = min(nk, kt + DIST) - (kt + 1);
            if (DIST >= 3 && younger == 2) dma_wait<2 * PER_TILE>();
            else if (DIST >= 2 && younger >= 1) dma_wait<(DIST >= 2 ? PER_TILE : 0)>();
            else dma_wait<0>();
            AA_TICK(0)
            block_barrier();
            AA_TICK(1)
            int issue_at = (STAGGER && wave >= NW / 2) ? KS / 2 : 0;
            if (STAGGER && (p.debug & 0x1000)) issue_at = (wave >= NW / 2) ? (p.debug >> 10) & 3 : (p.debug >> 8) & 3;
            const bool more = kt + DIST < nk && !(p.debug & 1);
            if (!(p.debug & 2)) compute(kt % STAGES, issue_at, kt + DIST, more);
            else if (more) issue(kt + DIST, (kt + DIST) % STAGES);
            if constexpr (SPREAD) { if (kt + 1 + DIST < nk) issue_prepare(kt + 1 + DIST, (kt + 1 + DIST) % STAGES); }
            AA_TICK(3)
        }
    }
#ifdef AA_PHASE_PROBE
    if ((p.debug & 8) && tid == 0)
        for (int k = 0; k < 4; ++k) reinterpret_cast<long long*>(p.workspace)[((int64_t)65536 + blockIdx.x) * 8 + k] = pt[k];
#endif
#undef AA_TICK

    stamp(2);
    const int ec = lane & 31, eh = lane >> 5;
    const int m_tile = m_begin + tile_m * BM;
    const int n_wave = tile_n * BN + wn * (BN / WN);
    if (k_splits > 1) {
        float* ws = reinterpret_cast<float*>(p.workspace) + ((int64_t)blockIdx.y * (M - m_begin) - m_begin) * p.n_pad;
#pragma unroll
        for (int i = 0; i < MI; ++i) {
            const int m = m_tile + wm * (BM / WM) + i * 32 + ec;
            if (m >= M) continue;
#pragma unroll
            for (int j = 0; j < NI; ++j) {
                float* dst = ws + (int64_t)m * p.n_pad + n_wave + j * 32 + 16 * eh;
#pragma unroll
                for (int q = 0; q < 4; ++q)
                    *reinterpret_cast<f32x4*>(dst + 4 * q) = f32x4{acc[i][j][4 * q], acc[i][j][4 * q + 1], acc[i][j][4 * q + 2], acc[i][j][4 * q + 3]};
            }
        }
        return;
    }

    cgd_epilogue<T, MI, NI>(p, M, acc, m_tile + wm * (BM / WM), n_wave, sBias + wn * (BN / WN));
    stamp(5);
}

}

namespace aa {
template <typename T>
__global__ void __launch_bounds__(256) splitk_reduce_kernel(const AaConvGemm p, const int M, const int m_begin, const int splits) {
    const int cpr = p.n_out >> 3;
    const int rows = M - m_begin;
    const int64_t total = (int64_t)rows * cpr;
    const float* ws = reinterpret_cast<const float*>(p.workspace);
    const T* bias = reinterpret_cast<const T*>(p.bias);
    const T* rowvec = reinterpret_cast<const T*>(p.rowvec);
    const T* resid = reinterpret_cast<const T*>(p.residual);
    T* out = reinterpret_cast<T*>(p.out);
    for (int64_t c = (int64_t)blockIdx.x * 256 + threadIdx.x; c < total; c += (int64_t)gridDim.x * 256) {
        const int ml = (int)(c / cpr), n = (int)(c - (int64_t)ml * cpr) * 8;
        const int m = m_begin + ml;
        float v[8];
#pragma unroll
        for (int e = 0; e < 8; ++e) v[e] = 0.0f;
        for (int sp = 0; sp < splits; ++sp) {
            const f32x4* src = reinterpret_cast<const f32x4*>(ws + ((int64_t)sp * rows + ml) * p.n_pad + n);
            const f32x4 a = src[0], b = src[1];
#pragma unroll
            for (int e = 0; e < 4; ++e) { v[e] += a[e]; v[4 + e] += b[e]; }
        }
        if (p.ln_stats) {
            const LnRow lr = cgd_ln_row(p, m);
            const float* cs = p.ln_cols + n;
#pragma unroll
            for (int e = 0; e < 8; ++e) v[e] = fmaf(v[e], lr.a, fmaf(lr.nm, cs[e], cs[p.n_pad + e]));
        }
        if (bias) {
#pragma unroll
            for (int e = 0; e < 8; ++e) v[e] += (float)bias[p.bias_per_row ? m : n + e];
// ... 26 lines not shown
```

### animate_anything_amd/csrc/kernels/conv_gemm_x.h

```cpp
#pragma once
#include "dev.h"
#include "aa_mi355.h"
#include "conv_gemm_dma.h"

namespace aa {

__host__ __device__ constexpr bool cgx_ln_ok(int bk, int wm, int wn, int per_cu) { return wm * wn * per_cu <= 4 && bk == 64; }
constexpr int CGX_COEF_BYTES = 4096;
__host__ __device__ inline int cgx_lds_main_bytes(int bm, int bn, int bk, int ring, int wm, int wn, int per_cu) {
    return cgd_lds_bytes(bm, bn, bk, ring) + (cgx_ln_ok(bk, wm, wn, per_cu) ? wm * wn * 2048 : 0);
}
__host__ __device__ inline int cgx_lds_bytes(int bm, int bn, int bk, int ring, int wm, int wn, int per_cu) {
    return cgx_lds_main_bytes(bm, bn, bk, ring, wm, wn, per_cu) + CGX_COEF_BYTES;
}

__host__ __device__ constexpr bool cgx_ticket_ok(int bm, int bn, int wm, int wn, int per_cu) {
    return (bm / wm / 32) * (bn / wn / 32) <= 4 || (bm == 192 && bn == 256 && (wm * wn * per_cu + 3) / 4 == 1);
}

template <typename T, int BM, int BN, int WM, int WN, int BK, int DP3, int DP0, int DP1, int RING = (BK == 64 ? 2 : 4), int PER_CU = 1, bool LIN = false>
__global__ void __launch_bounds__(64 * WM * WN, (PER_CU * WM * WN + 3) / 4) conv_gemm_x_kernel(const AaConvGemm p, const int M, const int tiles_n, const int m_begin, const int k_splits) {
    constexpr int STAGES = RING;
    static_assert(BK == 64 ? RING == 2 : (RING == 3 || RING == 4), "ring depth");
    constexpr int NW = WM * WN;
    constexpr int MI = BM / WM / 32;
    constexpr int NI = BN / WN / 32;
    constexpr int NB = MI * NI;
    constexpr int ROWB = BK * 2;
    constexpr int SPR = BK / 8;
    constexpr int RPI = 64 / SPR;
    constexpr int RPB = 256 / ROWB;
    constexpr int GA = BM / RPI, GB = BN / RPI;
    constexpr int AJ = (GA + NW - 1) / NW;
    constexpr int BJ = (GB + NW - 1) / NW;
    constexpr int PER_TILE = AJ + BJ;
    constexpr int DP2 = PER_TILE - DP3 - DP0 - DP1;
    constexpr int STAGE_BYTES = (BM + BN) * ROWB;
    constexpr int R = MI + NI;
    constexpr int KS = BK / 16;
    static_assert(BM % (32 * WM) == 0 && BN % (32 * WN) == 0 && BM % RPI == 0 && BN % RPI == 0, "tile shape");
    static_assert(NB <= ACC_BLOCKS && R <= NB, "accumulator file");
    static_assert(BK == 64 || BK == 32, "K step");
    static_assert(DP2 >= 0 && DP3 >= 0 && DP0 >= 0 && DP1 >= 0 && (BK == 64 || (DP0 == 0 && DP1 == 0)), "DMA schedule");
    static_assert(BN * 2 <= 1024, "bias slice");
    static_assert(AJ <= NB, "one activation row offset per MFMA gap of a sub-step");
    char* smem = dyn_smem();
    char* dummy = smem + STAGES * STAGE_BYTES;
    T* sBias = reinterpret_cast<T*>(dummy + 1024);

    const int tid = threadIdx.x;
    const int lane = tid & 63;
    const int wave = wave_id();
    const int wm = wave / WN, wn = wave % WN;

    const int nwg = gridDim.x, bid = blockIdx.x;
    const int q = nwg >> 3, r = nwg & 7;
    const int xcd = bid & 7, idx = bid >> 3;
    const int logical = (xcd < r ? xcd * (q + 1) : r * (q + 1) + (xcd - r) * q) + idx;
    int tile_m, tile_n;
    {
        const int tiles_m = nwg / tiles_n;
        const int a_tile_bytes = BM * (p.c0 + p.c1) * 2;
        int gm = ((p.debug & 16) || tiles_n < 8) ? 1 : min(8, max(1, (5 << 19) / a_tile_bytes));
        gm = min(gm, tiles_m);
        const int panel = gm * tiles_n, pidx = logical / panel;
        const int rows_here = min(gm, tiles_m - pidx * gm);
        const int within = logical - pidx * panel;
        tile_n = within / rows_here;
        tile_m = pidx * gm + (within - tile_n * rows_here);
    }

    auto stamp = [&](int slot) __attribute__((always_inline)) {
        if ((p.debug & 8) && tid == 0) reinterpret_cast<long long*>(p.workspace)[(int64_t)blockIdx.x * 8 + slot] = clock_now();
    };
    auto stamp_wall = [&](int slot, int id_slot) __attribute__((always_inline)) {
        if ((p.debug & 8) && tid == 0) {
            long long* w = reinterpret_cast<long long*>(p.workspace) + (int64_t)blockIdx.x * 8;
            w[slot] = wall_now();
            if (id_slot >= 0) w[id_slot] = hw_id();
        }
    };
    stamp(0);
    stamp_wall(7, 3);
    const int ctot = p.c0 + p.c1;
    const int nk_all = p.k_pad / BK;
    const int k_per = (nk_all + k_splits - 1) / k_splits;
    const int kbase = blockIdx.y * k_per;
    const int nk = max(0, min(k_per, nk_all - kbase));
    const bool linear = LIN || (p.kh * p.kw == 1 && p.stride == 1 && p.pad_h == 0 && p.pad_w == 0);
    const int kh_ = LIN ? 1 : p.kh, kw_ = LIN ? 1 : p.kw;

    constexpr unsigned OOB = 0x80000000u;
    const int margin_px = linear ? 0 : p.pad_h * p.w_in + p.pad_w;
    const BufRsrc r_a0 = make_rsrc(static_cast<const char*>(p.a0) - (int64_t)margin_px * p.c0 * 2, (unsigned)(((int64_t)p.n_img * p.h_in * p.w_in + margin_px) * p.c0 * 2));
    const BufRsrc r_a1 = make_rsrc(p.c1 ? static_cast<const char*>(p.a1) - (int64_t)margin_px * p.c1 * 2 : nullptr, p.c1 ? (unsigned)(((int64_t)p.n_img * p.h_in * p.w_in + margin_px) * p.c1 * 2) : 0u);
    const BufRsrc r_w = make_rsrc(p.w, (unsigned)((int64_t)p.n_pad * p.k_pad * 2));
    constexpr int swm = SPR - 1;
    const bool two_src = p.c1 != 0;
    const int lrow = lane / SPR, lpos = lane % SPR;
    unsigned pixi[AJ], inv[AJ];
    struct RowCoords { int img, iy, ix; bool ok; };
    auto row_coords = [&](int j) __attribute__((always_inline)) {
        const int rr = (wave + NW * j) * RPI + lrow;
        const int m = m_begin + tile_m * BM + rr;
        const bool ok = m < M && rr < BM;
        const int mm = ok ? m : 0;
        if (linear) return RowCoords{0, 0, mm, ok};
        const int x = mm % p.w_out;
        const int t = mm / p.w_out;
        const int y = t % p.h_out;
        return RowCoords{t / p.h_out, y * p.stride - p.pad_h, x * p.stride - p.pad_w, ok};
    };
    static_assert((RPI * NW / RPB) % SPR == 0, "the swizzle term must not depend on the piece index");
    const unsigned slot16 = (unsigned)((lpos ^ (((wave * RPI + lrow) / RPB) & swm)) * 16);
#pragma unroll
    for (int j = 0; j < AJ; ++j) {
        const RowCoords rc = row_coords(j);
        const int iy = rc.iy, ix = rc.ix;
        pixi[j] = (unsigned)((rc.img * p.h_in + iy) * p.w_in + ix + margin_px);
        const int ylo = max(0, -iy), yhi = max(ylo, min(kh_, p.h_virt - iy));
        const int xlo = max(0, -ix), xhi = max(xlo, min(kw_, p.w_virt - ix));
        const unsigned mx = ((1u << xhi) - 1u) ^ ((1u << xlo) - 1u);
        unsigned valid = 0u;
        for (int dy = ylo; dy < yhi; ++dy) valid |= mx << (dy * kw_);
        inv[j] = rc.ok ? ~valid : ~0u;
    }
    const unsigned wb0 = (unsigned)((tile_n * BN + wave * RPI + lrow) * p.k_pad) * 2u + slot16;
    const unsigned wb_step = (unsigned)(NW * RPI * p.k_pad) * 2u;
    const int taps = kh_ * kw_;

    int n_tap, n_dx, n_toff, n_cb;
    {
        const int k0 = kbase * BK;
        const int unit = k0 >> 6, chunk = unit / taps;
        n_tap = unit - chunk * taps;
        n_cb = chunk * 64 + (k0 & 63);
        const int dy = n_tap / kw_;
        n_dx = n_tap - dy * kw_;
        n_toff = dy * p.w_in + n_dx;
    }
    const int wrap_d = p.w_in - kw_ + 1;
    int cur_src = -1;
    unsigned pb[AJ];
    bool is_src1 = false;
    unsigned is_ccb = 0u, is_kb = 0u;
    int is_buf = 0;
    unsigned s_c2 = 0u, s_sh = 0u;
    unsigned v_t = 0u;
    auto prep_row = [&](auto j_) __attribute__((always_inline)) {
        constexpr int j = decltype(j_)::value;
        im2col_offset(pb[j], pixi[j], s_c2, v_t, s_sh, inv[j]);
    };
    auto prep_scalars = [&](int kt, int buf) __attribute__((always_inline)) {
        const int tap = n_tap, cb = n_cb, toff = n_toff;
        {
            const bool last_tap = n_tap + 1 == taps;
            const bool wrap_x = n_dx + 1 == kw_;
            const int t1 = last_tap ? 0 : n_tap + 1;
            const int o1 = last_tap ? 0 : n_toff + (wrap_x ? wrap_d : 1);
            const int x1 = (last_tap || wrap_x) ? 0 : n_dx + 1;
            if constexpr (BK == 32) {
                const bool stay = !(n_cb & 32);
                n_cb = stay ? n_cb + 32 : (n_cb & ~63) + (last_tap ? 64 : 0);
                n_tap = stay ? n_tap : t1; n_toff = stay ? n_toff : o1; n_dx = stay ? n_dx : x1;
            } else {
                n_cb += last_tap ? 64 : 0;
                n_tap = t1; n_toff = o1; n_dx = x1;
            }
        }
        is_src1 = cb >= p.c0;
        s_c2 = (unsigned)(is_src1 ? p.c1 : p.c0) * 2u;
        s_sh = (unsigned)(31 - min(tap, 31));
        v_t = slot16 + (unsigned)toff * s_c2;
        is_ccb = (unsigned)(is_src1 ? cb - p.c0 : cb) * 2u;
        is_kb = (unsigned)((kbase + kt) * BK) * 2u;
        is_buf = buf;
        if constexpr (LIN) {
            const int src = is_src1 ? 1 : 0;
            if (src != cur_src) { cur_src = src; static_for<AJ>(prep_row); }
        }
    };
    auto prepare = [&](int kt, int buf) __attribute__((always_inline)) {
        prep_scalars(kt, buf);
        if constexpr (!LIN) static_for<AJ>(prep_row);
    };
    auto dma_piece = [&](auto jj_) __attribute__((always_inline)) {
        constexpr int jj = decltype(jj_)::value;
        if constexpr (jj < AJ) {
            constexpr int j = jj;
            const bool real = (GA % NW == 0) || (wave + NW * j < GA);
            char* a = smem + is_buf * STAGE_BYTES + wave * RPI * ROWB;
            async_copy16_buf_s(is_src1 ? r_a1 : r_a0, real ? pb[j] : OOB, is_ccb, real ? a + j * NW * RPI * ROWB : dummy);
        } else {
            constexpr int j = jj - AJ;
            const bool real = (GB % NW == 0) || (wave + NW * j < GB);
            char* b = smem + is_buf * STAGE_BYTES + BM * ROWB + wave * RPI * ROWB;
            async_copy16_buf_s(r_w, real ? wb0 : OOB, is_kb + j * wb_step, real ? b + j * NW * RPI * ROWB : dummy);
        }
    };
    auto dma_range = [&](auto j0_, auto j1_) __attribute__((always_inline)) {
        constexpr int J0 = decltype(j0_)::value, J1 = decltype(j1_)::value;
        static_for<J1 - J0>([&](auto t) __attribute__((always_inline)) { dma_piece(IntTag<J0 + decltype(t)::value>()); });
    };

    const int frow = lane & 31, fh = lane >> 5;
    int a_off[MI], w_off[NI];
    auto fragment_offsets = [&]() __attribute__((always_inline)) {
#pragma unroll
        for (int i = 0; i < MI; ++i) { const int rr = wm * (BM / WM) + i * 32 + frow; a_off[i] = rr * ROWB + ((fh ^ ((rr / RPB) & swm)) << 4); }
        const int prow = (frow & 3) + 4 * (frow >> 3) + 16 * ((frow >> 2) & 1);
#pragma unroll
        for (int j = 0; j < NI; ++j) { const int rr = wn * (BN / WN) + j * 32 + prow; w_off[j] = BM * ROWB + rr * ROWB + ((fh ^ ((rr / RPB) & swm)) << 4); }
    };
    static_assert(STAGE_BYTES % ROWB == 0 && ROWB % 64 == 0 && (BM * ROWB) % 256 == 0, "XOR addressing of the k sub-steps");

    AccFile af;
    if constexpr (PER_CU > 1) wave_priority<2>();
    const bool bias_folded = k_splits == 1 && !p.bias_per_row;
    const BufRsrc r_bias = make_rsrc(p.bias, (p.bias && bias_folded) ? (unsigned)p.n_out * 2u : 0u);
    constexpr bool LN_OK = cgx_ln_ok(BK, WM, WN, PER_CU);
    const bool ln_start = LN_OK && p.ln_stats != nullptr && k_splits == 1;
    constexpr int LNW = BN / WN;
    float* sLnW = reinterpret_cast<float*>(dummy + 2048) + wave * 512;
    float ln_nmean[LN_OK ? MI : 1], ln_sd[LN_OK ? MI : 1], ln_rstd[LN_OK ? MI : 1];
    u32x4 bias_raw[NI][2];
    if (!ln_start) {
#pragma unroll
        for (int j = 0; j < NI; ++j)
#pragma unroll
            for (int q = 0; q < 2; ++q)
                bias_raw[j][q] = buf_load16(r_bias, (unsigned)(tile_n * BN + wn * (BN / WN) + j * 32 + 16 * (lane >> 5) + 8 * q) * 2u);
    }
    if constexpr (LN_OK) if (ln_start) {
        static_assert(!LN_OK || LNW * 4 <= 1024, "one LDS-DMA piece per column vector");
        const BufRsrc r_ln = make_rsrc(p.ln_cols, (unsigned)(2 * p.n_pad) * 4u);
        const unsigned c0b = (unsigned)(tile_n * BN + wn * LNW) * 4u + (unsigned)lane * 16u;
        const bool in = lane * 4 < LNW;
        async_copy16_buf(r_ln, in ? c0b : OOB, sLnW);
        async_copy16_buf(r_ln, in ? c0b + (unsigned)p.n_pad * 4u : OOB, sLnW + 256);
#pragma unroll
        for (int i = 0; i < MI; ++i) {
            const LnRow r = cgd_ln_row(p, min(m_begin + tile_m * BM + wm * (BM / WM) + i * 32 + (lane & 31), M - 1));
            ln_nmean[i] = r.nmean; ln_sd[i] = r.sd; ln_rstd[i] = r.a;
        }
    }
    auto start_from_bias = [&]() __attribute__((always_inline)) {
        static_for<NI>([&](auto j_) __attribute__((always_inline)) {
            constexpr int j = decltype(j_)::value;
            if (LN_OK && ln_start) {
              if constexpr (LN_OK) {
                f32x16 cs, bp;
#pragma unroll
                for (int q4 = 0; q4 < 4; ++q4) {
                    const f32x4 c4 = *reinterpret_cast<const f32x4*>(sLnW + j * 32 + 16 * (lane >> 5) + 4 * q4);
                    const f32x4 b4 = *reinterpret_cast<const f32x4*>(sLnW + 256 + j * 32 + 16 * (lane >> 5) + 4 * q4);
#pragma unroll
                    for (int e = 0; e < 4; ++e) { cs[4 * q4 + e] = c4[e]; bp[4 * q4 + e] = b4[e]; }
                }
                static_for<MI>([&](auto i_) __attribute__((always_inline)) {
                    constexpr int i = decltype(i_)::value;
                    f32x16 v;
#pragma unroll
                    for (int e = 0; e < 16; e += 2) {
                        const f32x2 t = f32x2{bp[e], bp[e + 1]} * f32x2{ln_sd[i], ln_sd[i]};
                        const f32x2 r = __builtin_elementwise_fma(f32x2{ln_nmean[i], ln_nmean[i]}, f32x2{cs[e], cs[e + 1]}, t);
                        v[e] = r[0]; v[e + 1] = r[1];
                    }
                    acc_init<i * NI + j>(af, v);
                });
              }
            } else {
                f32x16 b;
#pragma unroll
                for (int q = 0; q < 2; ++q) {
                    Pack8<T> h; h.raw = bias_raw[j][q];
#pragma unroll
                    for (int e = 0; e < 8; ++e) b[8 * q + e] = (float)h.e[e];
                }
                static_for<MI>([&](auto i_) __attribute__((always_inline)) { acc_init<decltype(i_)::value * NI + j>(af, b); });
            }
        });
    };

    u32x4 fa[2][MI], fw[2][NI];
    auto frag_read = [&](const char* st, auto ks_, auto set_, auto rd_) __attribute__((always_inline)) {
        constexpr int ks = decltype(ks_)::value, set = decltype(set_)::value, rd = decltype(rd_)::value;
        if constexpr (rd == 0)       lds_read16_xor(fa[set][0], st + a_off[0], IntTag<(ks << 5)>());
        else if constexpr (rd <= NI) lds_read16_xor(fw[set][rd - 1], st + w_off[rd - 1], IntTag<(ks << 5)>());
        else                         lds_read16_xor(fa[set][rd - NI], st + a_off[rd - NI], IntTag<(ks << 5)>());
    };
    auto substep = [&](auto ks_, auto ksn_, const char* st_rd, const bool do_read, auto dj0_, auto dn_, auto prep_) __attribute__((always_inline)) {
        constexpr int ks = decltype(ks_)::value, ksn = decltype(ksn_)::value, set = ks & 1;
        constexpr int DJ0 = decltype(dj0_)::value, DN = decltype(dn_)::value;
        constexpr bool PREP = decltype(prep_)::value && !LIN;
        constexpr int G0 = (DN <= NB - R) ? R : NB - DN;
        static_for<NB>([&](auto g_) __attribute__((always_inline)) {
            constexpr int g = decltype(g_)::value, i = g / NI, j = g % NI;
            acc_mfma<i * NI + j>(af, T(), fw[set][j], fa[set][i]);
            if constexpr (g < R) { if (do_read) frag_read(st_rd, IntTag<ksn>(), IntTag<set ^ 1>(), IntTag<g>()); }
            if constexpr (PREP && g < AJ) prep_row(IntTag<g>());
            if constexpr (DN > 0 && g >= G0 && g < G0 + DN) dma_piece(IntTag<DJ0 + g - G0>());
        });
        lds_wait_all();
    };
    auto kstep = [&](int kt, auto has_next_, auto has_next2_) __attribute__((always_inline)) {
        constexpr bool HAS_NEXT = decltype(has_next_)::value, HAS_NEXT2 = decltype(has_next2_)::value;
        const char* st = smem + (kt & 1) * STAGE_BYTES;
        const char* st_next = smem + ((kt + 1) & 1) * STAGE_BYTES;
        substep(IntTag<0>(), IntTag<1>(), st, true, IntTag<DP3>(), IntTag<HAS_NEXT ? DP0 : 0>(), BoolTag<false>());
        substep(IntTag<1>(), IntTag<2>(), st, true, IntTag<DP3 + DP0>(), IntTag<HAS_NEXT ? DP1 : 0>(), BoolTag<false>());
        substep(IntTag<2>(), IntTag<3>(), st, true, IntTag<DP3 + DP0 + DP1>(), IntTag<HAS_NEXT ? DP2 : 0>(), BoolTag<false>());
        if constexpr (HAS_NEXT) {
            if constexpr (!(AA_X_ABLATE & 64)) dma_wait<0>();
            if constexpr (!(AA_X_ABLATE & 32)) block_barrier();
        }
        if constexpr (HAS_NEXT2) prep_scalars(kt + 2, kt & 1);
        substep(IntTag<3>(), IntTag<0>(), st_next, HAS_NEXT, IntTag<0>(), IntTag<HAS_NEXT2 ? DP3 : 0>(), BoolTag<HAS_NEXT2>());
    };

    auto put_bias = [&](auto younger_) __attribute__((always_inline)) {
        if (tid < BN / 8) *reinterpret_cast<u32x4*>(sBias + tid * 8) = u32x4{0u, 0u, 0u, 0u};
        if constexpr (LN_OK) { if (ln_start) { dma_wait<decltype(younger_)::value>(); wave_sync(); } }
        start_from_bias();
    };
    if constexpr (BK == 64) {
        if (nk > 0) {
            prepare(0, 0);
            stamp(1);
// ... 159 lines not shown
```

### animate_anything_amd/layers.py

```python
from __future__ import annotations

from dataclasses import dataclass, replace
from typing import Optional

import os

import torch
import torch.nn as nn

from . import ops
from ._lib import AA_ACT_NONE, AA_ACT_SILU


@dataclass(frozen=True)
class Grid:
    clips: int
    frames: int
    h: int
    w: int

    @property
    def images(self):
        return self.clips * self.frames

    @property
    def hw(self):
        return self.h * self.w

    @property
    def tokens(self):
        return self.images * self.hw

    def resized(self, h, w):
        return replace(self, h=h, w=w)


def weights_key(*tensors):
    return tuple((t.data_ptr(), t._version) for t in tensors if t is not None)


class _Packed:
    _pw = None
    _pw_key = None

    def _apply(self, fn, *a, **k):
        self._pw = None
        return super()._apply(fn, *a, **k)

    def _load_from_state_dict(self, *a, **k):
        self._pw = None
        return super()._load_from_state_dict(*a, **k)

    def packed(self):
        key = weights_key(self.weight, self.bias)
        if self._pw is None or self._pw_key != key:
            self._pw, self._pw_key = ops.pack_weight(self.weight, self.bias), key
        return self._pw


LN_FOLD = True
LN_FOLD_FF = os.environ.get("AA_LN_FOLD_FF", "1") == "1"
FF_PROJ_MERGE = os.environ.get("AA_FF_PROJ_MERGE", "1") == "1"
SEQ_ATTN = os.environ.get("AA_SEQ_ATTN", "1") == "1"
SEQ_PRE = os.environ.get("AA_SEQ_PRE", "0") == "1"
FF_FUSED = os.environ.get("AA_FF_FUSED", "1") == "1"
FF_SPLIT = os.environ.get("AA_FF_SPLIT", "1") == "1"
SEQ_ATTN_CHANNELS = tuple(int(c) for c in os.environ.get("AA_SEQ_ATTN_CHANNELS", "320,512").split(",") if c)
LINEAR_ROWS = os.environ.get("AA_LINEAR_ROWS", "1") == "1"
GN_FOLD = os.environ.get("AA_GN_FOLD", "1") == "1"
AA_FP8_FF = os.environ.get("AA_FP8_FF", "0") == "1"
FP8_FF_MIN_DIM = 640
LINEAR_ROWS_MIN = 16384


def rows_path(channels, n_out, rows, dtype):
    return LINEAR_ROWS and rows >= LINEAR_ROWS_MIN and ops.linear_rows_ok(channels, n_out, rows, dtype)


UPSAMPLE_AS_PARITY_CONVS = True


def _no_eager(name):
    raise RuntimeError(f"{name}: this module only runs through the HIP token path of animate_anything_amd")


class Linear(_Packed, nn.Linear):
    _sp = None
    _sp_key = None

    _rp = None
    _rp_key = None

    def rows_packed(self):
        key = weights_key(self.weight, self.bias)
        if self._rp is None or self._rp_key != key:
            self._rp, self._rp_key = ops.pack_linear_rows(self.weight, self.bias), key
        return self._rp

    def tokens(self, x, affine=None, **epilogue):
        if affine is not None or (not epilogue.get("row_stats") and not (set(epilogue) - {"residual", "row_stats", "coef_eps"}) and x.dim() == 2
                                  and x.stride(1) == 1 and rows_path(self.in_features, self.out_features, x.shape[0], x.dtype) and x.shape[1] == self.in_features):
            return ops.linear_rows(x, self.rows_packed(), epilogue.get("residual"), affine=affine)
        return ops.conv_gemm(x, self.packed(), ops.linear_geom(x.shape[0]), **epilogue)

    def norm_rows_ok(self, x, tokens_per_group):
        return GN_FOLD and x.dim() == 2 and x.stride(1) == 1 and x.shape[1] == self.in_features and \
            rows_path(self.in_features, self.out_features, x.shape[0], x.dtype) and ops.linear_rows_ok(self.in_features, self.out_features, x.shape[0], x.dtype, tokens_per_group)

    def seq_pre(self):
        key = weights_key(self.weight, self.bias)
        if self._sp is None or self._sp_key != key:
            self._sp, self._sp_key = ops.pack_seq_pre(self.weight, self.bias), key
        return self._sp

    def _apply(self, fn, *a, **k):
        self._sp = None
        self._rp = None
        return super()._apply(fn, *a, **k)

    def forward(self, x):
        _no_eager("Linear")


class Conv2d(_Packed, nn.Conv2d):
    def tokens(self, x, geom, **epilogue):
        return ops.conv_gemm(x, self.packed(), geom, **epilogue)

    def forward(self, x):
        _no_eager("Conv2d")


class Conv3d(_Packed, nn.Conv3d):
    def tokens(self, x, geom, **epilogue):
        return ops.conv_gemm(x, self.packed(), geom, **epilogue)

    def forward(self, x):
        _no_eager("Conv3d")


class GroupNorm(nn.GroupNorm):
    def coef_tokens(self, x, n_stat_groups, tokens_per_group):
        return ops.groupnorm_coef(x, self.weight, self.bias, n_stat_groups, tokens_per_group, self.num_groups, self.eps)

    def tokens(self, x, n_stat_groups, tokens_per_group, silu=False, x1=None, out=None):
        return ops.groupnorm(x, self.weight, self.bias, n_stat_groups, tokens_per_group, self.num_groups,
                             self.eps, silu, x1=x1, out=out)

    def forward(self, x):
        _no_eager("GroupNorm")


class LayerNorm(nn.LayerNorm):
    def tokens(self, x):
        return ops.layernorm(x, self.weight, self.bias, self.eps)

    def forward(self, x):
        _no_eager("LayerNorm")


class TimestepEmbedding(nn.Module):

    def __init__(self, in_channels, time_embed_dim, cond_proj_dim=None, out_dim=None):
        super().__init__()
        self.linear_1 = Linear(in_channels, time_embed_dim)
        self.cond_proj = Linear(cond_proj_dim, in_channels, bias=False) if cond_proj_dim else None
        self.linear_2 = Linear(time_embed_dim, out_dim or time_embed_dim)

    def tokens(self, sample, condition=None, final_silu=False):
        if condition is not None:
            sample = self.cond_proj.tokens(condition, residual=sample)
        h = self.linear_1.tokens(sample, act=AA_ACT_SILU)
        return self.linear_2.tokens(h, act=AA_ACT_SILU if final_silu else AA_ACT_NONE)


class ResnetBlock2D(nn.Module):

    def __init__(self, in_channels, out_channels=None, temb_channels=1280, eps=1e-5, groups=32,
                 output_scale_factor=1.0):
        super().__init__()
        out_channels = out_channels or in_channels
        self.norm1 = GroupNorm(groups, in_channels, eps=eps)
        self.conv1 = Conv2d(in_channels, out_channels, 3, padding=1)
        self.time_emb_proj = Linear(temb_channels, out_channels) if temb_channels else None
        self.norm2 = GroupNorm(groups, out_channels, eps=eps)
        self.conv2 = Conv2d(out_channels, out_channels, 3, padding=1)
        self.conv_shortcut = Conv2d(in_channels, out_channels, 1) if in_channels != out_channels else None
        self.output_scale_factor = output_scale_factor
        self.tproj = None

    def tokens(self, x, g: Grid, temb_silu=None, x1=None):
        geom = ops.conv3x3_geom(g.images, g.h, g.w)
        h = self.norm1.tokens(x, g.images, g.hw, silu=True, x1=x1)
        if self.time_emb_proj is not None and temb_silu is not None:
            tproj = self.tproj if self.tproj is not None else self.time_emb_proj.tokens(temb_silu)
            self.tproj = None
            h = self.conv1.tokens(h, geom, rowvec=tproj, rowvec_div=g.frames * g.hw)
        else:
            h = self.conv1.tokens(h, geom)
        h = self.norm2.tokens(h, g.images, g.hw, silu=True)
        if self.conv_shortcut is not None:
            skip = self.conv_shortcut.tokens(x, ops.linear_geom(g.tokens), x1=x1)
        else:
            skip = x
        return self.conv2.tokens(h, geom, residual=skip, out_scale=1.0 / self.output_scale_factor)


class TemporalConvLayer(nn.Module):

    def __init__(self, in_dim, out_dim=None, dropout=0.0):
        super().__init__()
        out_dim = out_dim or in_dim

        def stage(cin, cout, with_dropout):
            mods = [GroupNorm(32, cin), nn.SiLU()] + ([nn.Dropout(dropout)] if with_dropout else [])
            return nn.Sequential(*mods, Conv3d(cin, cout, (3, 1, 1), padding=(1, 0, 0)))

        self.conv1 = stage(in_dim, out_dim, False)
        self.conv2 = stage(out_dim, in_dim, True)
        self.conv3 = stage(out_dim, in_dim, True)
        self.conv4 = stage(out_dim, in_dim, True)
        nn.init.zeros_(self.conv4[-1].weight)
        nn.init.zeros_(self.conv4[-1].bias)

    def tokens(self, x, g: Grid):
        geom = ops.tconv_geom(g.clips, g.frames, g.hw)
        h = x
        for i, seq in enumerate((self.conv1, self.conv2, self.conv3, self.conv4)):
            h = seq[0].tokens(h, g.clips, g.frames * g.hw, silu=True)
            h = seq[-1].tokens(h, geom, residual=x if i == 3 else None)
        return h


class Downsample2D(nn.Module):
    def __init__(self, channels, out_channels=None, padding=1):
        super().__init__()
        self.padding = padding
        self.conv = Conv2d(channels, out_channels or channels, 3, stride=2, padding=padding)

    def tokens(self, x, g: Grid):
        geom = ops.conv3x3_geom(g.images, g.h, g.w, stride=2, pad=self.padding)
        return self.conv.tokens(x, geom), g.resized(geom.h_out, geom.w_out)


class Upsample2D(nn.Module):

    def __init__(self, channels, out_channels=None):
        super().__init__()
        self.conv = Conv2d(channels, out_channels or channels, 3, padding=1)

    def parity_packed(self):
        key = weights_key(self.conv.weight, self.conv.bias)
        if self._pp is None or self._pp_key != key:
            self._pp, self._pp_key = ops.pack_upsample2x_weights(self.conv.weight, self.conv.bias), key
        return self._pp

    _pp = None
    _pp_key = None

    def _apply(self, fn, *a, **k):
        self._pp = None
        return super()._apply(fn, *a, **k)

    def tokens(self, x, g: Grid, output_size=None):
        up = (2 * g.h, 2 * g.w) if output_size is None else tuple(int(s) for s in output_size)
        c = x.shape[-1]
        if up == (2 * g.h, 2 * g.w) and c % 64 == 0 and self.conv.out_channels % 8 == 0 and UPSAMPLE_AS_PARITY_CONVS:
            out = torch.empty(g.images * up[0] * up[1], self.conv.out_channels, dtype=x.dtype, device=x.device)
            for (a, b), pw in self.parity_packed().items():
                geom = ops.Geom(g.images, g.h, g.w, g.h, g.w, 1, 1 - a, 1 - b)
                ops.conv_gemm(x, pw, geom, out=out, out_map=(2, 2, a, b))
            return out, g.resized(*up)
        geom = ops.conv3x3_geom(g.images, g.h, g.w, up_to=up)
        return self.conv.tokens(x, geom), g.resized(*up)


class Attention(nn.Module):

    def __init__(self, query_dim, cross_attention_dim=None, heads=8, dim_head=64):
        super().__init__()
        inner = heads * dim_head
        self.heads, self.dim_head, self.inner = heads, dim_head, inner
        self.is_cross = cross_attention_dim is not None
        kv_dim = cross_attention_dim or query_dim
        self.to_q = Linear(query_dim, inner, bias=False)
        self.to_k = Linear(kv_dim, inner, bias=False)
        self.to_v = Linear(kv_dim, inner, bias=False)
        self.to_out = nn.ModuleList([Linear(inner, query_dim), nn.Dropout(0.0)])
        self._fused = None
        self._fused_key = None
        self.kv = None

    def _apply(self, fn, *a, **k):
        self._fused = None
        self._fused_ln = None
        self._rows_ln = None
        self._seq_w = None
        return super()._apply(fn, *a, **k)

    def fused(self):
        rows = [self.to_k.weight, self.to_v.weight] if self.is_cross else \
               [self.to_q.weight, self.to_k.weight, self.to_v.weight]
        key = weights_key(*rows)
        if self._fused is None or self._fused_key != key:
            self._fused, self._fused_key = ops.pack_weight(torch.cat([r.detach() for r in rows], dim=0)), key
        return self._fused

    def fused_ln(self, norm):
        rows = [self.to_q.weight] if self.is_cross else [self.to_q.weight, self.to_k.weight, self.to_v.weight]
        key = weights_key(*rows, norm.weight, norm.bias)
        if self._fused_ln is None or self._fused_ln_key != key:
            self._fused_ln = ops.pack_weight(torch.cat([r.detach() for r in rows], dim=0), None, ln=(norm.weight, norm.bias, norm.eps))
            self._fused_ln_key = key
        return self._fused_ln

    def rows_ln(self, norm):
        rows = [self.to_q.weight] if self.is_cross else [self.to_q.weight, self.to_k.weight, self.to_v.weight]
        key = weights_key(*rows, norm.weight, norm.bias)
        if self._rows_ln is None or self._rows_ln_key != key:
            self._rows_ln = ops.pack_linear_rows(torch.cat([r.detach() for r in rows], dim=0), None, ln=(norm.weight, norm.bias, norm.eps))
            self._rows_ln_key = key
        return self._rows_ln

    def rows_ok(self, x):
        return self.to_q.bias is None and x.dim() == 2 and x.stride(1) == 1 and \
            rows_path(self.to_q.in_features, self.inner * (1 if self.is_cross else 3), x.shape[0], x.dtype)

    _rows_ln = None
    _rows_ln_key = None
    _fused_ln = None
    _fused_ln_key = None
    _seq_w = None
    _seq_w_key = None

    def seq_packed(self, norm):
        key = weights_key(self.to_q.weight, self.to_k.weight, self.to_v.weight, norm.weight, norm.bias)
        if self._seq_w is None or self._seq_w_key != key:
            self._seq_w = ops.pack_seq_qkv(self.to_q.weight, self.to_k.weight, self.to_v.weight, ln=(norm.weight, norm.bias, norm.eps))
            self._seq_w_key = key
        return self._seq_w

    def seq_ok(self, x, g: "Grid", temporal: bool):
        return (SEQ_ATTN and temporal and not self.is_cross and self.dim_head == 64 and self.inner == x.shape[1] == self.to_q.in_features
                and self.inner in SEQ_ATTN_CHANNELS and self.to_q.bias is None and ops.seq_self_attention_ok(self.inner, g.frames, x.shape[0], x.dtype))

    def seq_attention(self, x, norm, g: "Grid", pre=None, residual=None):
        return ops.seq_self_attention(x, self.seq_packed(norm), g.clips, g.hw, g.frames, (g.frames * g.hw, 1, g.hw), scale=float(self.dim_head) ** -0.5,
                                      pre=None if pre is None else pre.seq_pre(), residual=residual)

    def text_kv(self, text_tokens):
        if self.kv is not None:
            kv, self.kv = self.kv, None
            return kv
# ... 315 lines not shown
```

### animate_anything_amd/ops.py

```python
from __future__ import annotations

import ctypes as C
import math
import os
from dataclasses import dataclass
from typing import Optional

import torch

from . import _lib
from ._lib import (AA_ACT_GELU, AA_ACT_NONE, AA_ACT_QUICK_GELU, AA_ACT_SILU, AA_BF16, AA_F16, AA_F32, AaAttention, AaAttnOperand,
                   AaBlend, AaConvGemm, AaFFFused, AaLinearRows, AaLinearFp8, AaQuantRowsFp8, AaDdimStepTok, AaDpmStep, AaDpmStepTok, AaEulerStepTok, AaGroupNorm, AaPackFrames, AaPackLatents, AaSeqSelfAttn, AaUnipcStepTok, AaFreeU, AaCfgRescale)

_DT = {torch.float16: AA_F16, torch.bfloat16: AA_BF16, torch.float32: AA_F32}

TRACE = None

AUTOTUNE = True
LAST_STAMPS = None
GN_PLANS = None
MAX_OPERAND_BYTES = 1 << 31
FORCE_TILE = -1
ATTN_FLAGS = int(os.environ.get("AA_ATTN_FLAGS", "0"))
if ATTN_FLAGS & ~13:
# ... 116 lines not shown
    for i, (bm, bn, bk, _st) in enumerate(TILE_TABLE):
        if not lib.aa_conv_gemm_tile_ok(C.byref(d), i):
            continue
        out.append((i, 0))
        if TILE_TABLE.flags(i) & 1:
            continue
        if d.geglu or bm < 128:
            continue
        tiles = -(-rows // bm) * (d.n_pad // bn)
        slots = 256 * TILE_TABLE.per_cu(i)
        nk = d.k_pad // bk
        if tiles >= slots:
            continue
        fill1 = tiles / slots
        for sp in (2, 3, 4, 5, 6, 8):
            if nk // sp < 8:
                break
            wgs = tiles * sp
            fill = wgs / (-(-wgs // slots) * slots)
            if wgs <= 3 * slots and fill >= 0.8 and fill > fill1 + 0.1:
                out.append((i, sp))
    return out


AUTOTUNE_EVENTS = 0


def _autotune(lib, d, stream, key, rows, dev):
    global AUTOTUNE_EVENTS
    AUTOTUNE_EVENTS += 1
    cands = _tile_candidates(d, rows)
    if "stats" in key:
        def emits(c, sp):
            d.tile, d.k_splits = c, sp
            need = lib.aa_conv_gemm_workspace(C.byref(d))
            keep = (d.workspace, d.workspace_bytes)
            d.workspace, d.workspace_bytes = (C.c_void_p(1), need) if need else (None, 0)
            n = lib.aa_conv_gemm_row_stats_parts(C.byref(d))
            d.workspace, d.workspace_bytes = keep
            return n > 0
        cands = [c for c in cands if emits(*c)] or cands
    best = (-1, 0)
    if len(cands) == 1:
        best = cands[0]
    if len(cands) > 1:
        e0, e1 = torch.cuda.Event(enable_timing=True), torch.cuda.Event(enable_timing=True)
        ws_keep = (d.workspace, d.workspace_bytes)

        def timed(c, sp, reps, raw=False):
            d.tile, d.k_splits = c, sp
            need = lib.aa_conv_gemm_workspace(C.byref(d))
            ws = torch.empty(max(need // 4, 1), dtype=torch.float32, device=dev)
            d.workspace, d.workspace_bytes = C.c_void_p(ws.data_ptr()), need
            if lib.aa_conv_gemm(C.byref(d), stream) != 0:
                return None
            ts = []
            for _ in range(reps):
                e0.record()
                lib.aa_conv_gemm(C.byref(d), stream)
                e1.record()
                e1.synchronize()
                ts.append(e0.elapsed_time(e1))
            if raw:
                return ts
            ts.sort()
            return ts[len(ts) // 2] if reps > 5 else ts[1]

        first = sorted((t, c) for c in cands for t in [timed(c[0], c[1], 5)] if t is not None)
        finalists = [c for _, c in first[:4]]
        samples = {c: [] for c in finalists}
        for _ in range(3):
            for c in finalists:
                ts = timed(c[0], c[1], 7, raw=True)
                if ts is not None:
                    samples[c] += ts
        final = sorted((sorted(v)[len(v) // 2], c) for c, v in samples.items() if v)
        if final:
            best = final[0][1]
        d.workspace, d.workspace_bytes = ws_keep
    _tile_cache[key] = best
    return best


def _autotune_groupnorm(lib, d, ws, nbytes, stream, key):
    global AUTOTUNE_EVENTS
    info = (C.c_int32 * 4)()
    best = (0, 0)
    if lib.aa_groupnorm_plan(C.byref(d), info):
        AUTOTUNE_EVENTS += 1
        e0, e1 = torch.cuda.Event(enable_timing=True), torch.cuda.Event(enable_timing=True)

        def timed(two):
            lib.aa_set_groupnorm_two_pass(two)
            try:
                ts = []
                for i in range(9):
                    e0.record()
                    lib.aa_groupnorm(C.byref(d), C.c_void_p(ws.data_ptr()), nbytes, stream)
                    e1.record()
                    e1.synchronize()
                    if i >= 2:
                        ts.append(e0.elapsed_time(e1))
            finally:
                lib.aa_set_groupnorm_two_pass(0)
            ts.sort()
            return ts[len(ts) // 2]

        t1, t2 = timed(0), timed(1)
        best = (1, 0) if t2 < t1 else (0, 0)
    _tile_cache[key] = best
    return best


def _ptr(t: Optional[torch.Tensor]):
    return None if t is None else C.c_void_p(t.data_ptr())


def _check(*tensors):
    for t in tensors:
        if t is None:
            continue
        if not t.is_cuda and not _lib.host_pointers_ok():
            raise RuntimeError("animate_anything_amd ops run on the GPU only (tensor is on %s)" % t.device)
        if not t.is_contiguous():
            raise RuntimeError("animate_anything_amd ops need contiguous tensors")


def _stream(t: torch.Tensor):
    return C.c_void_p(torch.cuda.current_stream(t.device).cuda_stream) if t.is_cuda else None


def _run(fn, *args):
    rc = fn(*args)
    if rc != 0:
        raise RuntimeError("libaa_mi355: " + _lib.get().aa_last_error().decode())


def _round_up(x, m):
    return (x + m - 1) // m * m


@dataclass
class PackedWeight:
    w: torch.Tensor
    bias: Optional[torch.Tensor]
    n_out: int
    kh: int
    kw: int
    cin: int
    geglu: int = 0
    k_order: int = 0
    ln_cols: Optional[torch.Tensor] = None
    ln_eps: float = 0.0

    @property
    def n_pad(self):
        return self.w.shape[0]

    @property
    def k_pad(self):
        return self.w.shape[1]


def pack_weight(weight: torch.Tensor, bias: Optional[torch.Tensor] = None, geglu: bool = False, ln=None) -> PackedWeight:
    w = weight.detach()
    b_ln = None
    if ln is not None:
        gamma, beta, eps = ln
        assert w.dim() == 2, "the LayerNorm fold is for nn.Linear weights"
        wf = w.float()
        b_ln = wf @ beta.detach().float() + (0.0 if bias is None else bias.detach().float())
        w = (wf * gamma.detach().float()[None, :]).to(w.dtype)
        bias = None
    if w.dim() == 2:
        n, kh, kw, cin = w.shape[0], 1, 1, w.shape[1]
        w4 = w.reshape(n, 1, 1, cin)
    elif w.dim() == 4:
        n, cin, kh, kw = w.shape
        w4 = w.permute(0, 2, 3, 1)
    elif w.dim() == 5:
        n, cin, kh, kw = w.shape[0], w.shape[1], w.shape[2], 1
        assert w.shape[3] == 1 and w.shape[4] == 1
        w4 = w.reshape(n, cin, kh).permute(0, 2, 1).reshape(n, kh, 1, cin)
    else:
        raise ValueError("unsupported weight rank %d" % w.dim())
    cpad = _round_up(cin, 8)
    if cpad != cin:
        w4 = torch.nn.functional.pad(w4, (0, cpad - cin))
    k = kh * kw * cpad
    k_order = 0
    if kh * kw > 1 and cpad % 64 == 0 and n % 8 == 0:
        w4 = w4.reshape(n, kh * kw, cpad // 64, 64).permute(0, 2, 1, 3)
        k_order = 1
    w2 = w4.reshape(n, k)
    b = None if bias is None else bias.detach()
    if geglu:
        d = n // 2
        gran = 32
        assert d % gran == 0, "GEGLU inner width must be a multiple of 32"
        val = torch.arange(d, device=w.device).reshape(d // gran, 1, gran)
        src = torch.cat([val, val + d], dim=1).reshape(-1)
        w2 = w2[src]
        b = None if b is None else b[src]
        b_ln = None if b_ln is None else b_ln[src]
    n_pad, k_pad = _round_up(n, 64), _round_up(k, 64)
    out = torch.zeros(n_pad, k_pad, dtype=w.dtype, device=w.device)
    out[:n, :k] = w2
    if b is not None and geglu and n_pad != n:
        b = torch.nn.functional.pad(b, (0, n_pad - n))
    ln_cols, ln_eps = None, 0.0
    if ln is not None:
        ln_cols = torch.zeros(2, n_pad, dtype=torch.float32, device=w.device)
        ln_cols[0] = out.float().sum(dim=1)
        ln_cols[1, :n] = b_ln
        ln_eps = float(ln[2])
    return PackedWeight(out.contiguous(), None if b is None else b.contiguous(), n, kh, kw, cpad, gran if geglu else 0, k_order,
                        ln_cols, ln_eps)


def pack_upsample2x_weights(weight: torch.Tensor, bias: Optional[torch.Tensor] = None):
    n, c, kh, kw = weight.shape
    assert kh == 3 and kw == 3
    w = weight.detach().float()
    groups = {0: ((0,), (1, 2)), 1: ((0, 1), (2,))}
    out = {}
    for a in (0, 1):
        for b in (0, 1):
            f = torch.zeros(n, c, 2, 2, dtype=torch.float32, device=w.device)
            for r, dys in enumerate(groups[a]):
                for q, dxs in enumerate(groups[b]):
                    for dy in dys:
                        for dx in dxs:
                            f[:, :, r, q] += w[:, :, dy, dx]
            out[(a, b)] = pack_weight(f.to(weight.dtype), bias)
    return out


@dataclass
class RowStats:
    data: Optional[torch.Tensor]
    rows: int
    parts: int
    _coef: Optional[torch.Tensor] = None
    _coef_key: tuple = ()

    def coef(self, channels, eps):
        if self._coef is None or self._coef_key != (channels, eps):
            if self.data is None:
                raise RuntimeError("RowStats: finished coefficients for (channels, eps) = %r were asked for %r" % (self._coef_key, (channels, eps)))
            out = torch.empty(self.rows, 4, dtype=torch.float32, device=self.data.device)
            _run(_lib.get().aa_ln_finalize, _ptr(self.data), self.parts, _ptr(out), self.rows, channels, float(eps), _stream(self.data))
            self._coef, self._coef_key = out, (channels, eps)
        return self._coef

    def repeat(self, n):
        if self.data is None:
            return RowStats(None, self.rows * n, 0, torch.cat([self._coef] * n), self._coef_key)
        return RowStats(torch.cat([self.data] * n), self.rows * n, self.parts)


@dataclass
class Geom:
    n_img: int
    h_in: int
    w_in: int
    h_out: int
    w_out: int
    stride: int = 1
    pad_h: int = 0
    pad_w: int = 0
    h_virt: int = 0
    w_virt: int = 0

    @property
    def rows(self):
        return self.n_img * self.h_out * self.w_out


def linear_geom(rows: int) -> Geom:
    return Geom(1, 1, rows, 1, rows)


def conv3x3_geom(n, h, w, stride=1, pad=1, up_to=None) -> Geom:
    hv, wv = (h, w) if up_to is None else up_to
    if stride == 1:
        ho, wo = hv, wv
    elif pad == 1:
        ho, wo = (hv + 2 - 3) // stride + 1, (wv + 2 - 3) // stride + 1
    else:
        ho, wo = (hv + 1 - 3) // stride + 1, (wv + 1 - 3) // stride + 1
    return Geom(n, h, w, ho, wo, stride, pad, pad, hv, wv)


def tconv_geom(clips, frames, hw) -> Geom:
    return Geom(clips, frames, hw, frames, hw, 1, 1, 0)


def conv_gemm(x0: torch.Tensor, pw: PackedWeight, g: Geom, x1: Optional[torch.Tensor] = None,
              rowvec: Optional[torch.Tensor] = None, rowvec_div: int = 1,
              residual: Optional[torch.Tensor] = None, act: int = AA_ACT_NONE, out_dtype=None,
              out_scale: float = 1.0, bias_per_row: bool = False, out: Optional[torch.Tensor] = None,
              bias: Optional[torch.Tensor] = "packed", acc_scale: float = 1.0, out_map=None, ln_stats=None, row_stats: bool = False,
              coef_eps: Optional[float] = None):
    lib = _lib.get()
    osc = 1 if out_map is None else out_map[0] * out_map[1]
    if out_map is not None and (out is None or out.shape[0] != g.rows * osc):
        raise RuntimeError("conv_gemm: out_map needs `out` = the whole [n_img * h_out * sy * w_out * sx, N] grid")
    b = pw.bias if isinstance(bias, str) else bias
    _check(x0, x1, pw.w, b, residual, out)
    if rowvec is not None:
        if (not rowvec.is_cuda and not _lib.host_pointers_ok()) or rowvec.stride(-1) != 1:
            raise RuntimeError("conv_gemm: rowvec must be a GPU tensor with contiguous rows")
    c0 = x0.shape[-1]
    c1 = 0 if x1 is None else x1.shape[-1]
    n_cols_ = pw.n_out // 2 if pw.geglu else pw.n_out
    in_rows = g.n_img * g.h_in * g.w_in
    biggest = 2 * max(in_rows * max(c0, c1), g.rows * max(osc * (n_cols_ if out is None else out.stride(0)),
                                                          0 if residual is None else residual.stride(0)))
    if biggest >= MAX_OPERAND_BYTES and g.n_img > 1 and not bias_per_row:
        if out is None:
            out = torch.empty(g.rows, n_cols_, dtype=x0.dtype if out_dtype is None else out_dtype, device=x0.device)
        parts = min(g.n_img, -(-biggest // (MAX_OPERAND_BYTES // 2)))
        per = -(-g.n_img // parts)
        ri, ro = g.h_in * g.w_in, g.h_out * g.w_out
        for i0 in range(0, g.n_img, per):
            n = min(per, g.n_img - i0)
            gi = Geom(n, g.h_in, g.w_in, g.h_out, g.w_out, g.stride, g.pad_h, g.pad_w, g.h_virt, g.w_virt)
            rv = rowvec
            if rowvec is not None:
                assert (i0 * ro) % rowvec_div == 0 and ((i0 + n) * ro) % rowvec_div == 0 or i0 + n == g.n_img
                rv = rowvec[(i0 * ro) // rowvec_div:]
            ls = None
            if ln_stats is not None:
                if ln_stats.data is None:
                    ls = RowStats(None, n * ri, 0, ln_stats._coef[i0 * ri:(i0 + n) * ri], ln_stats._coef_key)
                else:
                    ls = RowStats(ln_stats.data[i0 * ri:(i0 + n) * ri], n * ri, ln_stats.parts)
            conv_gemm(x0[i0 * ri:(i0 + n) * ri], pw, gi, None if x1 is None else x1[i0 * ri:(i0 + n) * ri], rv, rowvec_div,
                      None if residual is None else residual[i0 * ro:(i0 + n) * ro], act, out_dtype, out_scale, False,
                      out[i0 * ro * osc:(i0 + n) * ro * osc], bias, acc_scale, out_map, ls)
        return (out, None) if row_stats else out
    if c0 + c1 != pw.cin:
        raise RuntimeError(f"conv_gemm: activation has {c0}+{c1} channels, weight expects {pw.cin}")
    n_cols = pw.n_out // 2 if pw.geglu else pw.n_out
    odt = x0.dtype if out_dtype is None else out_dtype
    if out is None:
        out = torch.empty(g.rows, n_cols, dtype=odt, device=x0.device)
    d = AaConvGemm()
    d.a0, d.a1, d.w, d.bias = _ptr(x0), _ptr(x1), _ptr(pw.w), _ptr(b)
    d.rowvec, d.residual, d.out = _ptr(rowvec), _ptr(residual), _ptr(out)
    d.c0, d.c1 = c0, c1
    d.n_img, d.h_in, d.w_in = g.n_img, g.h_in, g.w_in
    d.h_virt, d.w_virt = g.h_virt or g.h_in, g.w_virt or g.w_in
    d.h_out, d.w_out = g.h_out, g.w_out
    d.kh, d.kw, d.stride, d.pad_h, d.pad_w = pw.kh, pw.kw, g.stride, g.pad_h, g.pad_w
    d.n_out, d.n_pad, d.k_pad = pw.n_out, pw.n_pad, pw.k_pad
    d.rowvec_div = rowvec_div
    d.rowvec_ld = 0 if rowvec is None or rowvec.dim() < 2 else rowvec.stride(0)
    d.ldo = out.stride(0)
    d.ldr = 0 if residual is None else residual.stride(0)
    d.act, d.geglu, d.bias_per_row = act, int(pw.geglu), int(bias_per_row)
    d.dtype, d.out_dtype, d.out_scale = _DT[x0.dtype], _DT[odt], out_scale
    d.acc_scale = 0.0 if acc_scale == 1.0 else float(acc_scale)
    if out_map is not None:
        d.out_sy, d.out_sx, d.out_oy, d.out_ox = (int(v) for v in out_map)
    if ln_stats is not None:
        if pw.ln_cols is None or ln_stats.rows != g.rows:
            raise RuntimeError("conv_gemm: ln_stats needs weights packed with a folded LayerNorm and statistics of every row of x0")
        if ln_stats.data is None or LN_FINALIZE_LAUNCH or (ln_stats.parts not in (2, 10) and not LN_RAW_ANY_PARTS):
            d.ln_stats, d.ln_cols = _ptr(ln_stats.coef(c0, pw.ln_eps)), _ptr(pw.ln_cols)
        else:
            d.ln_stats, d.ln_cols = _ptr(ln_stats.data), _ptr(pw.ln_cols)
            d.ln_parts, d.ln_eps = ln_stats.parts, float(pw.ln_eps)
    elif pw.ln_cols is not None:
        raise RuntimeError("conv_gemm: these weights carry a folded LayerNorm: pass the row statistics of x0 (ln_stats)")
    if acc_scale == 0.0:
        raise ValueError("conv_gemm: acc_scale == 0 is not representable (0 means 1 in the C ABI)")
    d.k_order = pw.k_order
    d.debug = DEBUG_ABLATE
    tk = _ticket_array(x0) if USE_TICKETS else None
    if tk is not None:
        d.tickets, d.tickets_len = _ptr(tk), tk.numel()
    d.tile, d.k_splits = -1, K_SPLITS
    key = (d.dtype, g.n_img, g.h_in, g.w_in, d.h_virt, d.w_virt, g.h_out, g.w_out, g.stride, pw.kh, pw.kw, c0, c1,
           pw.n_out, d.geglu, residual is not None) + (("ln",) if ln_stats is not None else ()) + (("stats",) if row_stats else ())
    if TILE_PICKER is not None and FORCE_TILE < 0 and K_SPLITS == 0:
        cands = _tile_candidates(d, g.rows)
        d.tile, d.k_splits = TILE_PICKER(key, cands) if cands else (-1, 0)
    elif AUTOTUNE and x0.is_cuda and FORCE_TILE < 0 and K_SPLITS == 0:
        _load_default_tile_cache()
        choice = _tile_cache.get(key)
        aliased = any(t is not None and t.untyped_storage().data_ptr() == out.untyped_storage().data_ptr()
                      for t in (x0, x1, residual, rowvec))
        if choice is None and not aliased and not torch.cuda.is_current_stream_capturing():
            choice = _autotune(lib, d, _stream(x0), key, g.rows, x0.device)
        d.tile, d.k_splits = (-1, 0) if choice is None else choice
    if FORCE_TILE >= 0:
        d.tile = FORCE_TILE
    ws = None
    need = lib.aa_conv_gemm_workspace(C.byref(d))
    if DEBUG_ABLATE & 8:
        global LAST_STAMPS
        ws = LAST_STAMPS = torch.zeros(2, 1 << 16, 8, dtype=torch.int64, device=x0.device)
        d.workspace, d.workspace_bytes = _ptr(ws), ws.numel() * 8
    elif need:
        ws = torch.empty(need // 4, dtype=torch.float32, device=x0.device)
        d.workspace, d.workspace_bytes = _ptr(ws), need
    stats = None
    if row_stats:
        parts = lib.aa_conv_gemm_row_stats_parts(C.byref(d))
        if parts > 0 and coef_eps is not None and PRODUCER_COEF and lib.aa_conv_gemm_row_coef_ok(C.byref(d)):
            coef = torch.empty(g.rows, 4, dtype=torch.float32, device=x0.device)
            stats = RowStats(None, g.rows, 0, coef, (pw.n_out, float(coef_eps)))
            d.row_coef, d.row_coef_eps = _ptr(coef), float(coef_eps)
        elif parts > 0:
            stats = RowStats(torch.empty(g.rows, parts, 2, dtype=torch.float32, device=x0.device), g.rows, parts)
            d.row_stats, d.row_stats_parts = _ptr(stats.data), parts
    _run(lib.aa_conv_gemm, C.byref(d), _stream(x0))
    if TRACE is not None:
        TRACE.append((d, (x0, x1, pw, b, rowvec, residual, out, ws, stats, ln_stats)))
    return (out, stats) if row_stats else out


def groupnorm(x0: torch.Tensor, gamma: torch.Tensor, beta: torch.Tensor, n_groups_img: int,
              tokens_per_group: int, num_groups: int = 32, eps: float = 1e-5, silu: bool = False,
              x1: Optional[torch.Tensor] = None, out: Optional[torch.Tensor] = None) -> torch.Tensor:
    lib = _lib.get()
    _check(x0, x1, gamma, beta, out)
    c0 = x0.shape[-1]
    c1 = 0 if x1 is None else x1.shape[-1]
    y = torch.empty(n_groups_img * tokens_per_group, c0 + c1, dtype=x0.dtype, device=x0.device) if out is None else out
    d = AaGroupNorm()
    d.x0, d.x1, d.gamma, d.beta, d.y = _ptr(x0), _ptr(x1), _ptr(gamma), _ptr(beta), _ptr(y)
    d.c0, d.c1 = c0, c1
    d.n_groups_img, d.tokens_per_group, d.num_groups = n_groups_img, tokens_per_group, num_groups
    d.silu, d.dtype, d.eps = int(silu), _DT[x0.dtype], eps
    nbytes = lib.aa_groupnorm_workspace(C.byref(d))
    ws = torch.empty(max(nbytes // 4, 1), dtype=torch.float32, device=x0.device)
    two_pass = False
    if AUTOTUNE and x0.is_cuda:
        key = (-1, d.dtype, c0, c1, n_groups_img, tokens_per_group, num_groups, int(silu))
        _load_default_tile_cache()
        choice = _tile_cache.get(key)
        if choice is None and y.data_ptr() != x0.data_ptr() and not torch.cuda.is_current_stream_capturing():
            choice = _autotune_groupnorm(lib, d, ws, nbytes, _stream(x0), key)
        two_pass = bool(choice and choice[0])
    if two_pass:
        lib.aa_set_groupnorm_two_pass(1)
    try:
        if GN_PLANS is not None:
            info = (C.c_int32 * 4)()
            GN_PLANS.append(tuple(info) if lib.aa_groupnorm_plan(C.byref(d), info) else None)
        _run(lib.aa_groupnorm, C.byref(d), _ptr(ws), nbytes, _stream(x0))
    finally:
        if two_pass:
            lib.aa_set_groupnorm_two_pass(0)
    return y


def groupnorm_coef(x0: torch.Tensor, gamma: torch.Tensor, beta: torch.Tensor, n_groups_img: int, tokens_per_group: int, num_groups: int = 32,
                   eps: float = 1e-5) -> torch.Tensor:
    lib = _lib.get()
    _check(x0, gamma, beta)
    c0 = x0.shape[-1]
    d = AaGroupNorm()
    d.x0, d.x1, d.gamma, d.beta, d.y = _ptr(x0), None, _ptr(gamma), _ptr(beta), None
    d.c0, d.c1 = c0, 0
    d.n_groups_img, d.tokens_per_group, d.num_groups = n_groups_img, tokens_per_group, num_groups
    d.silu, d.dtype, d.eps = 0, _DT[x0.dtype], eps
    nbytes = lib.aa_groupnorm_workspace(C.byref(d))
    ws = torch.empty(max(nbytes // 4, 1), dtype=torch.float32, device=x0.device)
    coef = torch.empty(n_groups_img, 2, c0, dtype=torch.float32, device=x0.device)
    _run(lib.aa_groupnorm_coef, C.byref(d), _ptr(ws), nbytes, _ptr(coef), _stream(x0))
    return coef


def layernorm(x: torch.Tensor, gamma: torch.Tensor, beta: torch.Tensor, eps: float = 1e-5) -> torch.Tensor:
    lib = _lib.get()
    _check(x, gamma, beta)
    y = torch.empty_like(x)
    _run(lib.aa_layernorm, _ptr(x), _ptr(gamma), _ptr(beta), _ptr(y), x.shape[0], x.shape[1], eps,
         _DT[x.dtype], _stream(x))
    return y


def _operand(t: torch.Tensor, col0: int, outer_stride: int, inner_stride: int, pos_stride: int, outer_div: int = 1):
    o = AaAttnOperand()
    o.ptr, o.ld, o.col0 = _ptr(t), t.stride(0), col0
    o.outer_stride, o.inner_stride, o.pos_stride, o.outer_div = outer_stride, inner_stride, pos_stride, outer_div
    return o


def attention(q: torch.Tensor, q_col0: int, k: torch.Tensor, k_col0: int, v: torch.Tensor, v_col0: int,
              heads: int, n_outer: int, n_inner: int, q_len: int, kv_len: int,
              q_strides, kv_strides, kv_outer_div: int = 1, scale: Optional[float] = None, head_dim: int = 64,
              kv_seq_mod: int = 0, causal: bool = False) -> torch.Tensor:
    lib = _lib.get()
    for t in (q, k, v):
        if (not t.is_cuda and not _lib.host_pointers_ok()) or t.stride(-1) != 1:
            raise RuntimeError("attention: operands must be GPU tensors with contiguous rows")
    out = torch.empty(q.shape[0], heads * head_dim, dtype=q.dtype, device=q.device)
    d = AaAttention()
    d.q = _operand(q, q_col0, *q_strides)
    d.k = _operand(k, k_col0, *kv_strides, outer_div=kv_outer_div)
    d.v = _operand(v, v_col0, *kv_strides, outer_div=kv_outer_div)
    d.o = _operand(out, 0, *q_strides)
    d.k.seq_mod = d.v.seq_mod = kv_seq_mod
    d.causal = int(causal)
    d._pad = ATTN_FLAGS
    d.n_outer, d.n_inner, d.heads, d.head_dim = n_outer, n_inner, heads, head_dim
    d.q_len, d.kv_len, d.dtype = q_len, kv_len, _DT[q.dtype]
    d.scale = float(head_dim) ** -0.5 if scale is None else scale
    _run(lib.aa_attention, C.byref(d), _stream(q))
    return out


SEQ_ATTN_DEBUG = 0


@dataclass
class SeqQKV:
    w: torch.Tensor
    bias: Optional[torch.Tensor]
    ln_eps: float


def pack_seq_qkv(wq: torch.Tensor, wk: torch.Tensor, wv: torch.Tensor, ln=None) -> SeqQKV:
    n, c = wq.shape
    assert n % 64 == 0 and wk.shape == (n, c) and wv.shape == (n, c)
    i = torch.arange(32, device=wq.device)
    perm = 16 * ((i >> 2) & 1) + 4 * (i >> 3) + (i & 3)
    perm64 = torch.cat([perm, perm + 32])
    heads = n // 64

    def order(t):
        q, k, v = (t[j].reshape((heads, 64) + tuple(t.shape[2:])) for j in range(3))
        return torch.stack([k, v[:, perm64], q], dim=1).contiguous()

    w3 = torch.stack([wq.detach(), wk.detach(), wv.detach()])
    bias, eps = None, 0.0
    if ln is not None:
        gamma, beta, eps = ln
        wf = w3.float()
        bias = order(wf @ beta.detach().float())
        w3 = (wf * gamma.detach().float()[None, None, :]).to(wq.dtype)
    return SeqQKV(order(w3), bias, float(eps))


@dataclass
class SeqPre:
    w: torch.Tensor
    bias: Optional[torch.Tensor]


def pack_seq_pre(weight: torch.Tensor, bias: Optional[torch.Tensor] = None) -> SeqPre:
    n, c = weight.shape
    assert n == c and n % 64 == 0
    i = torch.arange(32, device=weight.device)
    perm = 16 * ((i >> 2) & 1) + 4 * (i >> 3) + (i & 3)
    rows = (torch.arange(0, n, 32, device=weight.device)[:, None] + perm[None, :]).reshape(-1)
    b = None if bias is None else bias.detach().float()[rows].contiguous()
    return SeqPre(weight.detach()[rows].reshape(n // 64, 64, c).contiguous(), b)


def _seq_self_attn_desc(x, pk, out, n_outer, n_inner, seq_len, strides, scale):
    d = AaSeqSelfAttn()
    d.x, d.w, d.w_bias, d.o = _ptr(x), _ptr(pk.w), _ptr(pk.bias), _ptr(out)
    d.outer_stride, d.inner_stride, d.pos_stride = strides
    last = (n_outer - 1) * strides[0] + (n_inner - 1) * strides[1] + (seq_len - 1) * strides[2]
    d.x_bytes, d.o_bytes = (last + 1) * x.stride(0) * 2, (last + 1) * out.stride(0) * 2
    d.n_outer, d.n_inner, d.seq_len, d.channels = n_outer, n_inner, seq_len, x.shape[1]
    d.ldx, d.ldo = x.stride(0), out.stride(0)
    d.normalize, d.ln_eps, d.scale, d.dtype = int(pk.ln_eps > 0.0), float(pk.ln_eps), float(scale), _DT[x.dtype]
# ... 541 lines not shown
```

### include/aa_mi355.h

```cpp
#ifndef AA_MI355_H
#define AA_MI355_H

#include <stddef.h>
#include <stdint.h>

#ifdef __cplusplus
extern "C" {
#endif

#define AA_VERSION 110

enum { AA_F16 = 0, AA_BF16 = 1, AA_F32 = 2 };
enum { AA_OK = 0, AA_E_SHAPE = -1, AA_E_DTYPE = -2, AA_E_ALIGN = -3, AA_E_WORKSPACE = -4, AA_E_HIP = -5 };
enum { AA_ACT_NONE = 0, AA_ACT_SILU = 1,
       AA_ACT_GELU = 2, AA_ACT_QUICK_GELU = 3  };

int aa_version(void);
const char* aa_last_error(void);

typedef struct AaConvGemm {
    const void* a0;
    const void* a1;
    const void* w;
    const void* bias;
    const void* rowvec;
    const void* residual;
    void* out;
    int32_t c0, c1;
    int32_t n_img, h_in, w_in, h_virt, w_virt, h_out, w_out;
    int32_t kh, kw, stride, pad_h, pad_w;
    int32_t n_out;
    int32_t n_pad, k_pad;
    int32_t rowvec_div;
    int32_t ldo, ldr;
    int32_t act;
    int32_t geglu;
    int32_t bias_per_row;
    int32_t dtype;
    int32_t out_dtype;
    float out_scale;
    void* workspace;
    int64_t workspace_bytes;
    int32_t k_order;
    int32_t debug;
    int32_t tile;
    int32_t k_splits;
    int32_t rowvec_ld;
    float acc_scale;
    int32_t out_sy, out_sx;
    int32_t out_oy, out_ox;
    const float* ln_stats;
    const float* ln_cols;
    int32_t ln_parts;
    float ln_eps;
    float* row_stats;
    int32_t row_stats_parts;
    int32_t tickets_len;
    int32_t* tickets;
    float* row_coef;
    float row_coef_eps;
    int32_t _reserved107;
} AaConvGemm;

size_t aa_conv_gemm_workspace(const AaConvGemm* d);
int aa_conv_gemm(const AaConvGemm* d, void* stream);
int aa_conv_gemm_launch_count(const AaConvGemm* d);
int aa_conv_gemm_tickets(const AaConvGemm* d);
int aa_conv_gemm_reduce_launches(const AaConvGemm* d);
int aa_conv_gemm_row_stats_parts(const AaConvGemm* d);
int aa_conv_gemm_row_coef_ok(const AaConvGemm* d);
int aa_ln_finalize(const float* stats, int32_t parts, float* coef, int64_t rows, int32_t channels, float eps, void* stream);

int aa_conv_gemm_tile_info(int idx, int32_t info[7]);

int aa_conv_gemm_tile_flags(int idx);

int aa_conv_gemm_tile_ok(const AaConvGemm* d, int idx);

void aa_set_tile_override(int cfg);

typedef struct AaGroupNorm {
    const void* x0;
    const void* x1;
    const void* gamma;
    const void* beta;
    void* y;
    int32_t c0, c1;
    int32_t n_groups_img;
    int32_t tokens_per_group;
    int32_t num_groups;
    int32_t silu;
    int32_t dtype;
    float eps;
} AaGroupNorm;

size_t aa_groupnorm_workspace(const AaGroupNorm* d);
void aa_set_groupnorm_two_pass(int on);
int aa_groupnorm_plan(const AaGroupNorm* d, int32_t info[4]);
int aa_groupnorm(const AaGroupNorm* d, void* workspace, size_t workspace_bytes, void* stream);
int aa_groupnorm_coef(const AaGroupNorm* d, void* workspace, size_t workspace_bytes, float* coef, void* stream);

int aa_layernorm(const void* x, const void* gamma, const void* beta, void* y,
                 int64_t rows, int32_t channels, float eps, int32_t dtype, void* stream);

typedef struct AaAttnOperand {
    const void* ptr;
    int64_t outer_stride, inner_stride, pos_stride;
    int32_t ld, col0, outer_div;
    int32_t seq_mod;
} AaAttnOperand;

typedef struct AaAttention {
    AaAttnOperand q, k, v, o;
    int32_t n_outer, n_inner, heads, head_dim;
    int32_t q_len, kv_len;
    int32_t dtype;
    float scale;
    int32_t causal;
    int32_t _pad;
} AaAttention;

int aa_attention(const AaAttention* d, void* stream);

typedef struct AaSeqSelfAttn {
    const void* x;
    const void* w;
    const float* w_bias;
    const void* pre_w;
    const float* pre_bias;
    const void* pre_residual;
    void* pre_out;
    void* o;
    int64_t outer_stride, inner_stride, pos_stride;
    int64_t x_bytes, o_bytes;
    int32_t n_outer, n_inner, seq_len;
    int32_t channels;
    int32_t ldx, ldo;
    int32_t ld_res, ld_pre;
    int32_t normalize;
    float ln_eps;
    float scale;
    int32_t dtype;
    int32_t flags;
} AaSeqSelfAttn;

int aa_seq_self_attention_ok(const AaSeqSelfAttn* d);
int aa_seq_self_attention(const AaSeqSelfAttn* d, void* stream);

#define AA_FF_STAGE_BYTES 41984
#define AA_FF_STAGES 65
typedef struct AaFFFused {
    const void* x;
    const void* outer;
    void* out;
    const void* w;
    int64_t rows;
    int32_t channels;
    int32_t ldx, ld_outer, ldo;
    int32_t normalize;
    float ln_eps;
    int32_t dtype;
    int32_t flags;
} AaFFFused;

int aa_ff_fused_ok(const AaFFFused* d);
int aa_ff_fused(const AaFFFused* d, void* stream);

#define AA_LR_STAGE_BYTES 21504
typedef struct AaLinearRows {
    const void* x;
    const void* residual;
    void* out;
    const void* w;
    int64_t rows;
    int32_t channels, n_out;
    int32_t ldx, ld_res, ldo;
    int32_t normalize;
    float ln_eps;
    int32_t dtype;
    int32_t flags;
    const float* row_affine;
    int32_t rows_per_group;
    int32_t _pad;
} AaLinearRows;

int aa_linear_rows_ok(const AaLinearRows* d);
int aa_linear_rows(const AaLinearRows* d, void* stream);

#define AA_FP8_TINY 1e-12f
typedef struct AaQuantRowsFp8 {
    const void* x;
    const void* gamma;
    const void* beta;
    void* q;
    float* scale;
    int64_t rows;
    int32_t channels;
    int32_t ldx;
    int32_t ldq;
    float ln_eps;
    int32_t dtype;
    int32_t _pad;
} AaQuantRowsFp8;

typedef struct AaLinearFp8 {
    const void* a;
    const float* a_scale;
    const void* w;
    const float* w_scale;
    const float* bias;
    const void* residual;
    void* out;
    int64_t rows;
    int32_t n, k;
// ... 185 lines not shown
```

Baseline: 16.62 steps/s.

## Merge ResNet 1x1 shortcut conv into conv2 GEMM as extra K tail

For ResNet blocks that have a 1x1 conv_shortcut, the shortcut weights are packed as extra K columns after conv2's 3x3 weights. The conv GEMM kernels (the X and DMA paths) switch their activation source to the block input for those tail K-steps at the centre tap, and the two biases are summed. This removes a separate shortcut GEMM launch and the write and read of its intermediate skip tensor. In exchange the packed weight grows, the slab path and tickets are disabled for these calls, and the new template instantiation may change register pressure.

```diff
diff --git a/animate_anything_amd/_lib.py b/animate_anything_amd/_lib.py
--- a/animate_anything_amd/_lib.py
+++ b/animate_anything_amd/_lib.py
@@ -25,6 +25,7 @@
         ("ln_stats", C.c_void_p), ("ln_cols", C.c_void_p), ("ln_parts", C.c_int32), ("ln_eps", C.c_float),
         ("row_stats", C.c_void_p), ("row_stats_parts", C.c_int32), ("tickets_len", C.c_int32), ("tickets", C.c_void_p),
         ("row_coef", C.c_void_p), ("row_coef_eps", C.c_float), ("_reserved107", C.c_int32),
+        ("t0", C.c_void_p), ("t1", C.c_void_p), ("tc0", C.c_int32), ("tc1", C.c_int32),
     ]
 
 
diff --git a/animate_anything_amd/csrc/aa_api_impl.h b/animate_anything_amd/csrc/aa_api_impl.h
--- a/animate_anything_amd/csrc/aa_api_impl.h
+++ b/animate_anything_amd/csrc/aa_api_impl.h
@@ -126,7 +126,9 @@
         if (taps > 1 && d.k_order != 1) return false;
         if (taps > 31) return false;
         const int64_t px = (int64_t)d.n_img * d.h_in * d.w_in + (int64_t)d.pad_h * d.w_in + d.pad_w + (int64_t)d.kh * d.w_in + d.kw;
-        if (px >= ((int64_t)1 << 24) || px * (d.c0 > d.c1 ? d.c0 : d.c1) * 2 >= ((int64_t)1 << 31)) return false;
+        int cmax = d.c0 > d.c1 ? d.c0 : d.c1;
+        if (d.tc0 > 0) { if (d.tc0 > cmax) cmax = d.tc0; if (d.tc1 > cmax) cmax = d.tc1; }
+        if (px >= ((int64_t)1 << 24) || px * cmax * 2 >= ((int64_t)1 << 31)) return false;
     }
     if (d.rowvec) {
         const int64_t M = (int64_t)d.n_img * d.h_out * d.w_out;
@@ -140,7 +142,7 @@
     const CgCfg& c = kCgCfgs[i];
     if (d.n_pad % c.bn) return false;
     if (d.geglu && (c.bn / c.wn) % 64) return false;
-    if (c.slab && !cg_slab_ok(d, c)) return false;
+    if (c.slab && (!cg_slab_ok(d, c) || d.tc0 > 0)) return false;
     if (c.x && (!cg_x_ok(d) || (i >= 36 && ((g_x_disabled >> (i - 36)) & 1u)))) return false;
     if (c.x && d.ln_stats && !cgx_ln_ok(c.bk, c.wm, c.wn, c.per_cu)) return false;
     return true;
@@ -182,6 +184,7 @@
            d.ldo % 8 == 0 && aligned16(d.out) && (!d.residual || (d.ldr % 8 == 0 && aligned16(d.residual))) &&
            d.n_out % 8 == 0 && (!d.bias || d.bias_per_row || aligned16(d.bias)) && (!d.rowvec || aligned16(d.rowvec)) &&
            (int64_t)d.n_img * d.h_in * d.w_in * (d.c0 > d.c1 ? d.c0 : d.c1) * 2 < ((int64_t)1 << 31) &&
+           (d.tc0 <= 0 || (int64_t)d.n_img * d.h_in * d.w_in * (d.tc0 > d.tc1 ? d.tc0 : d.tc1) * 2 < ((int64_t)1 << 31)) &&
            (int64_t)d.n_pad * d.k_pad * 2 < ((int64_t)1 << 31) &&
            (!cgd_out_mapped(d) || (int64_t)d.n_img * d.h_out * d.w_out * (d.out_sy > 1 ? d.out_sy : 1) * (d.out_sx > 1 ? d.out_sx : 1) * d.ldo * 2 < ((int64_t)1 << 31) - 32);
 }
@@ -263,7 +266,9 @@
 static void cg_launch_x(const AaConvGemm& d, int m_begin, int m_end, int splits, void* stream) {
     const int tiles_n = d.n_pad / BN;
     const dim3 grid(((m_end - m_begin + BM - 1) / BM) * tiles_n, splits), block(64 * WM * WN);
-    if (d.kh * d.kw == 1 && d.stride == 1 && d.pad_h == 0 && d.pad_w == 0)
+    if (d.tc0 > 0)
+        AA_LAUNCH((conv_gemm_x_kernel<T, BM, BN, WM, WN, BK, DP3, DP0, DP1, RING, PER_CU, false, true>), grid, block, cgx_lds_bytes(BM, BN, BK, RING, WM, WN, PER_CU), stream, d, m_end, tiles_n, m_begin, splits);
+    else if (d.kh * d.kw == 1 && d.stride == 1 && d.pad_h == 0 && d.pad_w == 0)
         AA_LAUNCH((conv_gemm_x_kernel<T, BM, BN, WM, WN, BK, DP3, DP0, DP1, RING, PER_CU, true>), grid, block, cgx_lds_bytes(BM, BN, BK, RING, WM, WN, PER_CU), stream, d, m_end, tiles_n, m_begin, splits);
     else
         AA_LAUNCH((conv_gemm_x_kernel<T, BM, BN, WM, WN, BK, DP3, DP0, DP1, RING, PER_CU, false>), grid, block, cgx_lds_bytes(BM, BN, BK, RING, WM, WN, PER_CU), stream, d, m_end, tiles_n, m_begin, splits);
@@ -603,6 +608,19 @@
     const int ctot = d->c0 + d->c1;
     if (d->c0 <= 0 || d->c0 % 8 || d->c1 % 8 || (d->c1 > 0 && !d->a1))
         return fail(AA_E_SHAPE, "conv_gemm: channels must be multiples of 8 (c0=%d c1=%d)", d->c0, d->c1);
+    if (d->tc0 != 0) {
+        const char* why = nullptr;
+        if (d->tc0 < 0 || d->tc0 % 64 || d->tc1 < 0 || d->tc1 % 64) why = "tc0 / tc1 must be multiples of 64";
+        else if (!d->t0 || (d->tc1 > 0 && !d->t1) || !aligned16(d->t0) || !aligned16(d->t1)) why = "t0 / t1 must be 16-byte aligned tensors";
+        else if (d->kh != 3 || d->kw != 3 || d->stride != 1 || d->pad_h != 1 || d->pad_w != 1 || d->h_virt != d->h_in || d->w_virt != d->w_in ||
+                 d->h_out != d->h_in || d->w_out != d->w_in) why = "a 3x3 / stride 1 / pad 1 convolution without a resize only";
+        else if (d->c1 != 0) why = "c1 must be 0";
+        else if (d->geglu || d->ln_stats || d->row_stats || d->row_coef || d->tickets || cgd_out_mapped(*d)) why = "no geglu / ln_stats / row_stats / row_coef / tickets / out_sy, out_sx > 1";
+        else if (d->out_dtype != d->dtype) why = "16-bit output";
+        else if (d->k_pad != 9 * d->c0 + d->tc0 + d->tc1) why = "k_pad must be 9 * c0 + tc0 + tc1";
+        else if (!cg_dma_ok(*d)) why = "needs the LDS-DMA path (channels % 64 == 0, 16-byte rows, < 2 GiB)";
+        if (why) return fail(AA_E_SHAPE, "conv_gemm: tail sources (tc0=%d tc1=%d): %s", d->tc0, d->tc1, why);
+    }
     if (d->n_pad % 64 || d->k_pad % CG_BK || d->k_pad < d->kh * d->kw * ctot || d->n_out > d->n_pad)
         return fail(AA_E_SHAPE, "conv_gemm: bad packed extents n_pad=%d k_pad=%d (K=%d, n_out=%d)", d->n_pad, d->k_pad, d->kh * d->kw * ctot, d->n_out);
     if (d->n_img <= 0 || d->h_out <= 0 || d->w_out <= 0 || d->kh <= 0 || d->kw <= 0 || d->stride <= 0 || d->rowvec_div <= 0)
diff --git a/animate_anything_amd/csrc/kernels/conv_gemm_dma.h b/animate_anything_amd/csrc/kernels/conv_gemm_dma.h
--- a/animate_anything_amd/csrc/kernels/conv_gemm_dma.h
+++ b/animate_anything_amd/csrc/kernels/conv_gemm_dma.h
@@ -414,8 +414,8 @@
     const bool linear = p.kh * p.kw == 1 && p.stride == 1 && p.pad_h == 0 && p.pad_w == 0 && !resize;
 
     constexpr unsigned OOB = 0x80000000u;
-    const BufRsrc r_a0 = make_rsrc(p.a0, (unsigned)((int64_t)p.n_img * p.h_in * p.w_in * p.c0 * 2));
-    const BufRsrc r_a1 = make_rsrc(p.a1, p.c1 ? (unsigned)((int64_t)p.n_img * p.h_in * p.w_in * p.c1 * 2) : 0u);
+    BufRsrc r_a0 = make_rsrc(p.a0, (unsigned)((int64_t)p.n_img * p.h_in * p.w_in * p.c0 * 2));
+    BufRsrc r_a1 = make_rsrc(p.a1, p.c1 ? (unsigned)((int64_t)p.n_img * p.h_in * p.w_in * p.c1 * 2) : 0u);
     const BufRsrc r_w = make_rsrc(p.w, (unsigned)((int64_t)p.n_pad * p.k_pad * 2));
 #ifdef AA_PHASE_PROBE
     const int swm = (p.debug & 16) ? 0 : SPR - 1;
@@ -471,12 +471,19 @@
         n_dy = n_tap / p.kw; n_dx = n_tap - n_dy * p.kw;
     }
     int cur_tap = -1;
+    constexpr int TAIL_TAP = 1 << 20;
+    const int t_c0 = p.tc0, t_c1 = p.tc1;
+    const void* const t_p0 = p.t0;
+    const void* const t_p1 = p.t1;
+    const int tail_k = t_c0 > 0 ? taps * ctot : 0x7fffffff;
     unsigned pb0[AJ], pb1[AJ];
     bool is_src1 = false;
     unsigned is_ccb = 0u, is_kb = 0u;
     int is_buf = 0;
-    auto issue_prepare = [&](int kt, int buf) {
-        const int tap = n_tap, cb = n_cb, dy = n_dy, dx = n_dx;
+    auto issue_prepare = [&](int kt, int buf) __attribute__((always_inline)) {
+        const int kpos = (kbase + kt) * BK;
+        const bool tail = kpos >= tail_k;
+        const int tap = tail ? TAIL_TAP : n_tap, cb = n_cb, dy = n_dy, dx = n_dx;
         {
             const bool wrap_x = n_dx + 1 == p.kw;
             if (p.k_order) {
@@ -496,7 +503,20 @@
                 n_dx = last_c ? (wrap_x ? 0 : n_dx + 1) : n_dx;
             }
         }
-        if (tap != cur_tap) {
+        if (tail && tap != cur_tap) {
+            cur_tap = tap;
+            r_a0 = make_rsrc(t_p0, (unsigned)((int64_t)p.n_img * p.h_in * p.w_in * t_c0 * 2));
+            r_a1 = make_rsrc(t_p1, t_c1 ? (unsigned)((int64_t)p.n_img * p.h_in * p.w_in * t_c1 * 2) : 0u);
+#pragma unroll
+            for (int j = 0; j < AJ; ++j) {
+                const int rr = (wave + NW * j) * RPI + lrow;
+                const int m = m_begin + tile_m * BM + rr;
+                const bool ok = m < M && rr < BM;
+                const int slot8 = (lpos ^ ((rr / RPB) & swm)) * 8;
+                pb0[j] = ok ? (unsigned)(m * t_c0 + slot8) * 2u : OOB;
+                pb1[j] = ok ? (unsigned)(m * t_c1 + slot8) * 2u : OOB;
+            }
+        } else if (tap != cur_tap) {
             cur_tap = tap;
             const bool tap_ok = tap < taps;
             if (!resize) {
@@ -529,12 +549,13 @@
                 }
             }
         }
-        is_src1 = cb >= p.c0;
-        is_ccb = (unsigned)(is_src1 ? cb - p.c0 : cb) * 2u;
-        is_kb = (unsigned)((kbase + kt) * BK) * 2u;
+        const int w0 = tail ? t_c0 : p.c0, ch = tail ? kpos - tail_k : cb;
+        is_src1 = ch >= w0;
+        is_ccb = (unsigned)(is_src1 ? ch - w0 : ch) * 2u;
+        is_kb = (unsigned)kpos * 2u;
         is_buf = buf;
     };
-    auto issue_dma = [&](auto j0_, auto j1_) {
+    auto issue_dma = [&](auto j0_, auto j1_) __attribute__((always_inline)) {
         constexpr int J0 = decltype(j0_)::value, J1 = decltype(j1_)::value;
         const BufRsrc ra = is_src1 ? r_a1 : r_a0;
         char* a = smem + is_buf * STAGE_BYTES + wave * RPI * ROWB;
@@ -552,7 +573,7 @@
             }
         }
     };
-    auto issue = [&](int kt, int buf) {
+    auto issue = [&](int kt, int buf) __attribute__((always_inline)) {
         issue_prepare(kt, buf);
         issue_dma(IntTag<0>(), IntTag<PER_TILE>());
     };
@@ -577,14 +598,14 @@
     auto frag_ptr_b = [&](const char* st, int ks, int j) { return st + b_off[j] + (((ks * 2 + fh) ^ b_swz[j]) << 4); };
     constexpr int KS = BK / 16;
     constexpr int SP = (KS >= 4 && STAGES == 2) ? KS - 1 : KS;
-    auto issue_piece = [&](auto ks_, int kt_next) {
+    auto issue_piece = [&](auto ks_, int kt_next) __attribute__((always_inline)) {
         constexpr int ks = decltype(ks_)::value;
         if constexpr (ks < SP) {
             constexpr int J0 = PER_TILE * ks / SP, J1 = PER_TILE * (ks + 1) / SP;
             issue_dma(IntTag<J0>(), IntTag<J1>());
         }
     };
-    auto compute = [&](int buf, int issue_at, int kt_next, bool more) {
+    auto compute = [&](int buf, int issue_at, int kt_next, bool more) __attribute__((always_inline)) {
         const char* st = smem + buf * STAGE_BYTES;
         if constexpr (FRAG_ASM) {
             u32x4 fa[2][MI], fb[2][NI];
diff --git a/animate_anything_amd/csrc/kernels/conv_gemm_x.h b/animate_anything_amd/csrc/kernels/conv_gemm_x.h
--- a/animate_anything_amd/csrc/kernels/conv_gemm_x.h
+++ b/animate_anything_amd/csrc/kernels/conv_gemm_x.h
@@ -18,7 +18,7 @@
     return (bm / wm / 32) * (bn / wn / 32) <= 4 || (bm == 192 && bn == 256 && (wm * wn * per_cu + 3) / 4 == 1);
 }
 
-template <typename T, int BM, int BN, int WM, int WN, int BK, int DP3, int DP0, int DP1, int RING = (BK == 64 ? 2 : 4), int PER_CU = 1, bool LIN = false>
+template <typename T, int BM, int BN, int WM, int WN, int BK, int DP3, int DP0, int DP1, int RING = (BK == 64 ? 2 : 4), int PER_CU = 1, bool LIN = false, bool TAIL = false>
 __global__ void __launch_bounds__(64 * WM * WN, (PER_CU * WM * WN + 3) / 4) conv_gemm_x_kernel(const AaConvGemm p, const int M, const int tiles_n, const int m_begin, const int k_splits) {
     constexpr int STAGES = RING;
     static_assert(BK == 64 ? RING == 2 : (RING == 3 || RING == 4), "ring depth");
@@ -44,6 +44,7 @@
     static_assert(DP2 >= 0 && DP3 >= 0 && DP0 >= 0 && DP1 >= 0 && (BK == 64 || (DP0 == 0 && DP1 == 0)), "DMA schedule");
     static_assert(BN * 2 <= 1024, "bias slice");
     static_assert(AJ <= NB, "one activation row offset per MFMA gap of a sub-step");
+    static_assert(!(LIN && TAIL), "tail sources ride on a 3x3 convolution");
     char* smem = dyn_smem();
     char* dummy = smem + STAGES * STAGE_BYTES;
     T* sBias = reinterpret_cast<T*>(dummy + 1024);
@@ -92,8 +93,12 @@
 
     constexpr unsigned OOB = 0x80000000u;
     const int margin_px = linear ? 0 : p.pad_h * p.w_in + p.pad_w;
-    const BufRsrc r_a0 = make_rsrc(static_cast<const char*>(p.a0) - (int64_t)margin_px * p.c0 * 2, (unsigned)(((int64_t)p.n_img * p.h_in * p.w_in + margin_px) * p.c0 * 2));
-    const BufRsrc r_a1 = make_rsrc(p.c1 ? static_cast<const char*>(p.a1) - (int64_t)margin_px * p.c1 * 2 : nullptr, p.c1 ? (unsigned)(((int64_t)p.n_img * p.h_in * p.w_in + margin_px) * p.c1 * 2) : 0u);
+    const int64_t src_px = (int64_t)p.n_img * p.h_in * p.w_in + margin_px;
+    auto src_rsrc = [&](const void* base, int ch) __attribute__((always_inline)) {
+        return make_rsrc(ch ? static_cast<const char*>(base) - (int64_t)margin_px * ch * 2 : nullptr, ch ? (unsigned)(src_px * ch * 2) : 0u);
+    };
+    BufRsrc r_a0 = src_rsrc(p.a0, p.c0);
+    BufRsrc r_a1 = src_rsrc(p.a1, p.c1);
     const BufRsrc r_w = make_rsrc(p.w, (unsigned)((int64_t)p.n_pad * p.k_pad * 2));
     constexpr int swm = SPR - 1;
     const bool two_src = p.c1 != 0;
@@ -140,6 +145,12 @@
         n_toff = dy * p.w_in + n_dx;
     }
     const int wrap_d = p.w_in - kw_ + 1;
+    const int t_c0 = TAIL ? p.tc0 : 0, t_c1 = TAIL ? p.tc1 : 0, m_c0 = p.c0, m_c1 = p.c1;
+    const void* const t_p0 = TAIL ? p.t0 : nullptr;
+    const void* const t_p1 = TAIL ? p.t1 : nullptr;
+    const unsigned tail_kb = TAIL ? (unsigned)(taps * ctot) * 2u : 0xffffffffu;
+    const int ctr_tap = p.pad_h * kw_ + p.pad_w, ctr_toff = margin_px;
+    bool in_tail = false;
     int cur_src = -1;
     unsigned pb[AJ];
     bool is_src1 = false;
@@ -152,7 +163,17 @@
         im2col_offset(pb[j], pixi[j], s_c2, v_t, s_sh, inv[j]);
     };
     auto prep_scalars = [&](int kt, int buf) __attribute__((always_inline)) {
-        const int tap = n_tap, cb = n_cb, toff = n_toff;
+        is_kb = (unsigned)((kbase + kt) * BK) * 2u;
+        const bool tail = TAIL && is_kb >= tail_kb;
+        const int tcb = TAIL ? (int)(is_kb - tail_kb) >> 1 : 0;
+        const int tap = tail ? ctr_tap : n_tap, cb = n_cb, toff = tail ? ctr_toff : n_toff;
+        if constexpr (TAIL) {
+            if (tail && !in_tail) {
+                in_tail = true;
+                r_a0 = src_rsrc(t_p0, t_c0);
+                r_a1 = src_rsrc(t_p1, t_c1);
+            }
+        }
         {
             const bool last_tap = n_tap + 1 == taps;
             const bool wrap_x = n_dx + 1 == kw_;
@@ -168,12 +189,12 @@
                 n_tap = t1; n_toff = o1; n_dx = x1;
             }
         }
-        is_src1 = cb >= p.c0;
-        s_c2 = (unsigned)(is_src1 ? p.c1 : p.c0) * 2u;
+        const int w0 = tail ? t_c0 : m_c0, w1 = tail ? t_c1 : m_c1, ch = tail ? tcb : cb;
+        is_src1 = ch >= w0;
+        s_c2 = (unsigned)(is_src1 ? w1 : w0) * 2u;
         s_sh = (unsigned)(31 - min(tap, 31));
         v_t = slot16 + (unsigned)toff * s_c2;
-        is_ccb = (unsigned)(is_src1 ? cb - p.c0 : cb) * 2u;
-        is_kb = (unsigned)((kbase + kt) * BK) * 2u;
+        is_ccb = (unsigned)(is_src1 ? ch - w0 : ch) * 2u;
         is_buf = buf;
         if constexpr (LIN) {
             const int src = is_src1 ? 1 : 0;
diff --git a/animate_anything_amd/layers.py b/animate_anything_amd/layers.py
--- a/animate_anything_amd/layers.py
+++ b/animate_anything_amd/layers.py
@@ -61,6 +61,7 @@
 LN_FOLD = True
 LN_FOLD_FF = os.environ.get("AA_LN_FOLD_FF", "1") == "1"
 FF_PROJ_MERGE = os.environ.get("AA_FF_PROJ_MERGE", "1") == "1"
+SHORTCUT_MERGE = os.environ.get("AA_SHORTCUT_MERGE", "1") == "1"
 SEQ_ATTN = os.environ.get("AA_SEQ_ATTN", "1") == "1"
 SEQ_PRE = os.environ.get("AA_SEQ_PRE", "0") == "1"
 FF_FUSED = os.environ.get("AA_FF_FUSED", "1") == "1"
@@ -188,6 +189,24 @@
         self.output_scale_factor = output_scale_factor
         self.tproj = None
 
+    _mp = None
+    _mp_key = None
+
+    def _apply(self, fn, *a, **k):
+        self._mp = None
+        return super()._apply(fn, *a, **k)
+
+    def merged_packed(self):
+        c2, cs = self.conv2, self.conv_shortcut
+        key = weights_key(c2.weight, c2.bias, cs.weight, cs.bias)
+        if self._mp is None or self._mp_key != key:
+            self._mp, self._mp_key = ops.pack_weight_tail(c2.weight, c2.bias, cs.weight, cs.bias), key
+        return self._mp
+
+    def shortcut_merged(self, x, x1=None):
+        return SHORTCUT_MERGE and self.conv_shortcut is not None and x.shape[-1] % 64 == 0 and (x1 is None or x1.shape[-1] % 64 == 0) and \
+            self.conv2.in_channels % 64 == 0 and self.conv2.out_channels % 8 == 0
+
     def tokens(self, x, g: Grid, temb_silu=None, x1=None):
         geom = ops.conv3x3_geom(g.images, g.h, g.w)
         h = self.norm1.tokens(x, g.images, g.hw, silu=True, x1=x1)
@@ -198,6 +217,8 @@
         else:
             h = self.conv1.tokens(h, geom)
         h = self.norm2.tokens(h, g.images, g.hw, silu=True)
+        if self.shortcut_merged(x, x1):
+            return ops.conv_gemm(h, self.merged_packed(), geom, out_scale=1.0 / self.output_scale_factor, tail=(x, x1))
         if self.conv_shortcut is not None:
             skip = self.conv_shortcut.tokens(x, ops.linear_geom(g.tokens), x1=x1)
         else:
diff --git a/animate_anything_amd/ops.py b/animate_anything_amd/ops.py
--- a/animate_anything_amd/ops.py
+++ b/animate_anything_amd/ops.py
@@ -292,6 +292,7 @@
     k_order: int = 0
     ln_cols: Optional[torch.Tensor] = None
     ln_eps: float = 0.0
+    tail: int = 0
 
     @property
     def n_pad(self):
@@ -358,6 +359,23 @@
                         ln_cols, ln_eps)
 
 
+def pack_weight_tail(weight: torch.Tensor, bias: Optional[torch.Tensor], tail_weight: torch.Tensor, tail_bias: Optional[torch.Tensor]) -> PackedWeight:
+    n, c, kh, kw = weight.shape
+    wt = tail_weight.detach().reshape(tail_weight.shape[0], -1)
+    ct = wt.shape[1]
+    if (kh, kw) != (3, 3) or c % 64 or ct % 64 or n % 8 or wt.shape[0] != n:
+        raise ValueError("pack_weight_tail: a 3x3 convolution over a multiple of 64 channels and a tail of a multiple of 64 channels")
+    main = pack_weight(weight, None)
+    assert main.k_order == 1 and main.k_pad == 9 * c
+    out = torch.zeros(main.n_pad, 9 * c + ct, dtype=main.w.dtype, device=main.w.device)
+    out[:, :9 * c] = main.w
+    out[:n, 9 * c:] = wt.to(main.w.dtype)
+    b = None
+    if bias is not None or tail_bias is not None:
+        b = sum(t.detach().float() for t in (bias, tail_bias) if t is not None).to(weight.dtype).contiguous()
+    return PackedWeight(out.contiguous(), b, n, 3, 3, c, 0, 1, None, 0.0, ct)
+
+
 def pack_upsample2x_weights(weight: torch.Tensor, bias: Optional[torch.Tensor] = None):
     n, c, kh, kw = weight.shape
     assert kh == 3 and kw == 3
@@ -441,13 +459,18 @@
               residual: Optional[torch.Tensor] = None, act: int = AA_ACT_NONE, out_dtype=None,
               out_scale: float = 1.0, bias_per_row: bool = False, out: Optional[torch.Tensor] = None,
               bias: Optional[torch.Tensor] = "packed", acc_scale: float = 1.0, out_map=None, ln_stats=None, row_stats: bool = False,
-              coef_eps: Optional[float] = None):
+              coef_eps: Optional[float] = None, tail=None):
     lib = _lib.get()
     osc = 1 if out_map is None else out_map[0] * out_map[1]
     if out_map is not None and (out is None or out.shape[0] != g.rows * osc):
         raise RuntimeError("conv_gemm: out_map needs `out` = the whole [n_img * h_out * sy * w_out * sx, N] grid")
     b = pw.bias if isinstance(bias, str) else bias
-    _check(x0, x1, pw.w, b, residual, out)
+    t0, t1 = (None, None) if tail is None else tail
+    _check(x0, x1, pw.w, b, residual, out, t0, t1)
+    tc0 = 0 if t0 is None else t0.shape[-1]
+    tc1 = 0 if t1 is None else t1.shape[-1]
+    if tc0 + tc1 != pw.tail or (tc1 and not tc0):
+        raise RuntimeError(f"conv_gemm: tail sources have {tc0}+{tc1} channels, the packed weight carries {pw.tail}")
     if rowvec is not None:
         if (not rowvec.is_cuda and not _lib.host_pointers_ok()) or rowvec.stride(-1) != 1:
             raise RuntimeError("conv_gemm: rowvec must be a GPU tensor with contiguous rows")
@@ -455,7 +478,7 @@
     c1 = 0 if x1 is None else x1.shape[-1]
     n_cols_ = pw.n_out // 2 if pw.geglu else pw.n_out
     in_rows = g.n_img * g.h_in * g.w_in
-    biggest = 2 * max(in_rows * max(c0, c1), g.rows * max(osc * (n_cols_ if out is None else out.stride(0)),
+    biggest = 2 * max(in_rows * max(c0, c1, tc0, tc1), g.rows * max(osc * (n_cols_ if out is None else out.stride(0)),
                                                           0 if residual is None else residual.stride(0)))
     if biggest >= MAX_OPERAND_BYTES and g.n_img > 1 and not bias_per_row:
         if out is None:
@@ -478,7 +501,8 @@
                     ls = RowStats(ln_stats.data[i0 * ri:(i0 + n) * ri], n * ri, ln_stats.parts)
             conv_gemm(x0[i0 * ri:(i0 + n) * ri], pw, gi, None if x1 is None else x1[i0 * ri:(i0 + n) * ri], rv, rowvec_div,
                       None if residual is None else residual[i0 * ro:(i0 + n) * ro], act, out_dtype, out_scale, False,
-                      out[i0 * ro * osc:(i0 + n) * ro * osc], bias, acc_scale, out_map, ls)
+                      out[i0 * ro * osc:(i0 + n) * ro * osc], bias, acc_scale, out_map, ls,
+                      tail=None if tail is None else (t0[i0 * ro:(i0 + n) * ro], None if t1 is None else t1[i0 * ro:(i0 + n) * ro]))
         return (out, None) if row_stats else out
     if c0 + c1 != pw.cin:
         raise RuntimeError(f"conv_gemm: activation has {c0}+{c1} channels, weight expects {pw.cin}")
@@ -518,12 +542,14 @@
         raise ValueError("conv_gemm: acc_scale == 0 is not representable (0 means 1 in the C ABI)")
     d.k_order = pw.k_order
     d.debug = DEBUG_ABLATE
-    tk = _ticket_array(x0) if USE_TICKETS else None
+    if tc0:
+        d.t0, d.t1, d.tc0, d.tc1 = _ptr(t0), _ptr(t1), tc0, tc1
+    tk = _ticket_array(x0) if USE_TICKETS and not tc0 else None
     if tk is not None:
         d.tickets, d.tickets_len = _ptr(tk), tk.numel()
     d.tile, d.k_splits = -1, K_SPLITS
     key = (d.dtype, g.n_img, g.h_in, g.w_in, d.h_virt, d.w_virt, g.h_out, g.w_out, g.stride, pw.kh, pw.kw, c0, c1,
-           pw.n_out, d.geglu, residual is not None) + (("ln",) if ln_stats is not None else ()) + (("stats",) if row_stats else ())
+           pw.n_out, d.geglu, residual is not None) + (("ln",) if ln_stats is not None else ()) + (("stats",) if row_stats else ()) + (("tail", tc0, tc1) if tc0 else ())
     if TILE_PICKER is not None and FORCE_TILE < 0 and K_SPLITS == 0:
         cands = _tile_candidates(d, g.rows)
         d.tile, d.k_splits = TILE_PICKER(key, cands) if cands else (-1, 0)
@@ -531,7 +557,7 @@
         _load_default_tile_cache()
         choice = _tile_cache.get(key)
         aliased = any(t is not None and t.untyped_storage().data_ptr() == out.untyped_storage().data_ptr()
-                      for t in (x0, x1, residual, rowvec))
+                      for t in (x0, x1, residual, rowvec, t0, t1))
         if choice is None and not aliased and not torch.cuda.is_current_stream_capturing():
             choice = _autotune(lib, d, _stream(x0), key, g.rows, x0.device)
         d.tile, d.k_splits = (-1, 0) if choice is None else choice
@@ -558,7 +584,7 @@
             d.row_stats, d.row_stats_parts = _ptr(stats.data), parts
     _run(lib.aa_conv_gemm, C.byref(d), _stream(x0))
     if TRACE is not None:
-        TRACE.append((d, (x0, x1, pw, b, rowvec, residual, out, ws, stats, ln_stats)))
+        TRACE.append((d, (x0, x1, pw, b, rowvec, residual, out, ws, stats, ln_stats, t0, t1)))
     return (out, stats) if row_stats else out
 
 
diff --git a/include/aa_mi355.h b/include/aa_mi355.h
--- a/include/aa_mi355.h
+++ b/include/aa_mi355.h
@@ -60,6 +60,9 @@
     float* row_coef;
     float row_coef_eps;
     int32_t _reserved107;
+    const void* t0;
+    const void* t1;
+    int32_t tc0, tc1;
 } AaConvGemm;
 
 size_t aa_conv_gemm_workspace(const AaConvGemm* d);
```

Result: no change. 16.66 steps/s (median of 6 runs) (+0.2%).
